# hengdashi/cuda_gcn

Measured on AMD Instinct MI355X. Metric: epochs_per_sec, higher is better.
Workload: dtype f32

## Files before the change

cuda_gcn_amd/_lib.py:

```python
from __future__ import annotations

import ctypes as C
import os

HERE = os.path.dirname(os.path.abspath(__file__))
LIBDIR = os.environ.get("GCN_LIBDIR") or os.path.join(HERE, "lib")

_cache = {}


class NativeLibraryMissing(RuntimeError):
    pass


def _load(name: str) -> C.CDLL:
    if name in _cache:
        return _cache[name]
    path = os.path.join(LIBDIR, name)
    if not os.path.exists(path):
        raise NativeLibraryMissing(
            f"{path} not found: the HIP extension is not built. Run `make kernels host` "
            f"(or __graft_entry__.build()); there is no CPU fallback.")
    try:
        lib = C.CDLL(path)
# ... 33 lines not shown

GCNHIP_SYMBOLS = {
    "gcnhip_device_count": (I, [C.POINTER(I)]),
    "gcnhip_ctx_create": (I, [C.POINTER(P), I, P]),
    "gcnhip_ctx_destroy": (I, [P]),
    "gcnhip_ctx_sync": (I, [P]),
    "gcnhip_ctx_set_corun": (I, [P, I]),
    "gcnhip_ctx_set_option": (I, [P, C.c_char_p, I]),
    "gcnhip_ctx_get_option": (I, [P, C.c_char_p, C.POINTER(I)]),
    "gcnhip_ctx_stream": (P, [P]),
    "gcnhip_error_string": (C.c_char_p, [I]),
    "gcnhip_last_error": (C.c_char_p, []),
    "gcnhip_version": (C.c_char_p, []),
    "gcnhip_experiments": (I, []),
    "gcnhip_malloc": (I, [P, C.POINTER(P), C.c_size_t]),
    "gcnhip_free": (I, [P, P]),
    "gcnhip_memset_async": (I, [P, P, I, C.c_size_t]),
    "gcnhip_h2d": (I, [P, P, P, C.c_size_t]),
    "gcnhip_d2h": (I, [P, P, P, C.c_size_t]),
    "gcnhip_d2d_async": (I, [P, P, P, C.c_size_t]),
    "gcnhip_host_alloc": (I, [C.POINTER(P), C.c_size_t]),
    "gcnhip_host_free": (I, [P]),
    "gcnhip_d2h_async": (I, [P, P, P, C.c_size_t]),
    "gcnhip_graph_create": (I, [P, C.POINTER(P), P, P, I, I, P]),
    "gcnhip_graph_create_grouped": (I, [P, C.POINTER(P), P, P, I, I, P, P]),
    "gcnhip_graph_set_schedule": (I, [P, P, I, P, I]),
    "gcnhip_graph_reserve_width": (I, [P, P, I]),
    "gcnhip_graph_destroy": (I, [P, P]),
    "gcnhip_graph_arrays": (I, [P, C.POINTER(P), C.POINTER(P), C.POINTER(P), C.POINTER(I), C.POINTER(I)]),
    "gcnhip_graphsum": (I, [P, P, P, I, P, I, I]),
    "gcnhip_graphsum_rowmask": (I, [P, P, P, I, P, I, I, P]),
    "gcnhip_graphsum_masked": (I, [P, P, P, I, P, I, I, P, P]),
    "gcnhip_graph_add_rowset": (I, [P, P, P, C.POINTER(P)]),
    "gcnhip_graph_create_restricted": (I, [P, C.POINTER(P), P, P]),
    "gcnhip_graph_clone": (I, [P, C.POINTER(P), P]),
    "gcnhip_rowset_size": (I, [P, C.POINTER(I)]),
    "gcnhip_graphsum_rowset": (I, [P, P, P, P, I, P, I, I, P]),
    "gcnhip_graphsum_relu_dropout": (I, [P, P, P, I, P, I, I, I, F, U64, P, U64, P]),
    "gcnhip_graphsum_relu_dropout_bits": (I, [P, P, P, I, P, I, I, I, F, U64, P, U64, P, P, I]),
    "gcnhip_graphsum_ex": (I, [P, P, P, P, I, P, I, I]),
    "gcnhip_graphsum_predict": (I, [P, P, P, P, P, I, P, I, I, I, P, P, P, I]),
    "gcnhip_graphsum_blend": (I, [P, P, P, I, P, I, P, I, I, F, F, F, F, P]),
    "gcnhip_cs_error_rows": (I, [P, P, I, P, I, P, I, I, P, I, P]),
    "gcnhip_cs_correct_rows": (I, [P, P, I, P, I, P, I, I, P, P, I]),
    "gcnhip_calib_nll_rows": (I, [P, P, I, P, I, P, I, I, F, P]),
    "gcnhip_calib_bins_rows": (I, [P, P, I, P, I, P, I, I, F, I, P, P, P]),
    "gcnhip_calib_scale_rows": (I, [P, P, I, I, P, I, I, F, P, I, P]),
    "gcnhip_conformal_scores": (I, [P, P, I, I, P, I, I, F, I, F, I, P, I]),
    "gcnhip_conformal_true_scores": (I, [P, P, I, P, I, P, I, I, P]),
    "gcnhip_conformal_sets_rows": (I, [P, P, I, I, P, I, I, P, P, P, P, P]),
    "gcnhip_sort_tile": (I, []),
    "gcnhip_rank_keys": (I, [P, P, I, I, P, I, I, I, I, P, P, I, P, P, I64, P, P, P, P]),
    "gcnhip_sort_segments_u32": (I, [P, P, P, I, I, I64]),
    "gcnhip_rank_stats": (I, [P, P, P, I64, I, I, P, P, P, P, P]),
    "gcnhip_embed_inv_norms": (I, [P, P, I, I, I, P]),
    "gcnhip_topk_plan": (I, [I, I, I, I, C.POINTER(I), C.POINTER(I), C.POINTER(C.c_size_t), C.POINTER(C.c_size_t)]),
    "gcnhip_topk_rows": (I, [P, P, I, I, I, P, P, P, I, I, I, I, P, C.c_size_t, I, P, P]),
    "gcnhip_pair_scores": (I, [P, P, I, I, I, P, P, P, I, P]),
    "gcnhip_embed_rows": (I, [P, P, I, I, I, P, P, I, P, I]),
    "gcnhip_explain_hops": (I, [P, P, P, P, I, P, I, I, P, I, I, I, P, P, I, P, P, P, I64]),
    "gcnhip_explain_features_agg": (I, [P, P, P, P, I, P, I, I, P, I, I, P, I, I, P, I, I, P, I]),
    "gcnhip_explain_features_walk": (I, [P, P, P, P, P, I, P, I, I, P, I, I, P, I, I, P, I]),
    "gcnhip_explain_abs_colsum": (I, [P, P, I, P, I, I, I, P, P]),
    "gcnhip_graph_remove_rowset": (I, [P, P, P]),
    "gcnhip_graph_scales": (I, [P, C.POINTER(P), C.POINTER(P), C.POINTER(P), C.POINTER(P)]),
    "gcnhip_feat_scale_rows": (I, [P, P, P]),
    "gcnhip_xent_fwd_rows_scaled": (I, [P, P, I, P, I, P, P, I, I, I, I, I, P, P, P]),
    "gcnhip_xent_from_row_terms": (I, [P, P, P, P, I, P, P]),
    "gcnhip_matmul_bwd_ex": (I, [P, P, I, P, I, P, I, P, I, P, I, I, I, I, F, P, I, P]),
    "gcnhip_graphsum_part": (I, [P, P, P, P, I, P, I, I, P, I, I, I, F, U64, P, U64, P]),
    "gcnhip_feat_create": (I, [P, C.POINTER(P), P, P, P, I, I]),
    "gcnhip_feat_create_aggregated": (I, [P, C.POINTER(P), P, P]),
    "gcnhip_feat_destroy": (I, [P, P]),
    "gcnhip_feat_is_dense": (I, [P]),
    "gcnhip_feat_values": (P, [P]),
    "gcnhip_feat_nnz": (I64, [P]),
    "gcnhip_spmm_fwd": (I, [P, P, P, P, I, P, I, I, F, U64, P, U64, P]),
    "gcnhip_spmm_fwd_relu": (I, [P, P, P, P, I, P, I, I]),
    "gcnhip_spmm_fwd_relu_matmul": (I, [P, P, P, P, I, I, P, I, I, P, I]),
    "gcnhip_spmm_bwd": (I, [P, P, P, P, I, P, I, I, F, U64, P, U64, P]),
    "gcnhip_spmm_bwd_plan": (I, [P, P, I, C.POINTER(I), C.POINTER(I)]),
    "gcnhip_spmm_bwd_part": (I, [P, P, P, P, I, I, F, U64, P, U64, P, I, I, I]),
    "gcnhip_spmm_bwd_finish": (I, [P, P, P, I, I]),
    "gcnhip_matmul_fwd": (I, [P, P, I, P, I, P, I, I, I, I]),
    "gcnhip_matmul_bwd": (I, [P, P, I, P, I, P, I, P, I, P, I, I, I, I]),
    "gcnhip_matmul_bwd_fused": (I, [P, P, I, P, I, P, I, P, I, P, I, I, I, I, F]),
    "gcnhip_matmul_bwd_fused_bits": (I, [P, P, I, P, I, P, I, P, I, P, I, I, I, I, F, P, I]),
    "gcnhip_pack_positive": (I, [P, P, I, I, I, P, I]),
    "gcnhip_f32_to_bf16": (I, [P, P, I, P, I, I64, I]),
    "gcnhip_graphsum_bf16": (I, [P, P, P, I, P, I, I, P, P, I, I, F, U64, P, U64, P]),
    "gcnhip_matmul_bwd_da_bits": (I, [P, P, I, P, I, P, I, I, I, I, P, I, F]),
    "gcnhip_gather_rows": (I, [P, P, I, P, I, P]),
    "gcnhip_relu_fwd": (I, [P, P, P, I64, I]),
    "gcnhip_relu_bwd": (I, [P, P, P, I64]),
    "gcnhip_dropout_fwd": (I, [P, P, P, I64, F, U64, P, U64, P]),
    "gcnhip_dropout_bwd": (I, [P, P, P, I64, F]),
    "gcnhip_relu_fwd_2d": (I, [P, P, I, I, I, P, I]),
    "gcnhip_relu_bwd_2d": (I, [P, P, I, I, I, P]),
    "gcnhip_dropout_fwd_2d": (I, [P, P, I, I, I, P, F, U64, P, U64, P]),
    "gcnhip_dropout_bwd_2d": (I, [P, P, I, I, I, P, F]),
    "gcnhip_relu_dropout_bwd": (I, [P, P, I, P, I, I, I, F]),
    "gcnhip_xent_fwd": (I, [P, P, I, P, I, P, I, I, I, I, I, P, P]),
    "gcnhip_xent_fwd_rows": (I, [P, P, I, P, I, P, P, I, I, I, I, I, P, P]),
    "gcnhip_accuracy": (I, [P, P, I, P, I, I, P]),
    "gcnhip_set_truth": (I, [P, P, P, P, I, I]),
    "gcnhip_sumsq": (I, [P, P, I64, P]),
    "gcnhip_adam_step": (I, [P, C.POINTER(AdamVar), I, F, P, P, F, F, F, F, P]),
    "gcnhip_adam_step_advance": (I, [P, C.POINTER(AdamVar), I, F, P, P, F, F, F, F, P, P, P]),
    "gcnhip_counter_add": (I, [P, P, C.c_uint32]),
    "gcnhip_metrics_record": (I, [P, P, I, I, P, P, P, P]),
    "gcnhip_metrics_record_with_next_loss": (I, [P, P, I, I, P, P]),
    "gcnhip_capture_begin": (I, [P]),
    "gcnhip_capture_end": (I, [P, C.POINTER(P)]),
    "gcnhip_graph_launch": (I, [P, P]),
    "gcnhip_graph_exec_destroy": (I, [P]),
    "gcnhip_event_create": (I, [C.POINTER(P)]),
    "gcnhip_event_create_sync": (I, [C.POINTER(P)]),
    "gcnhip_event_destroy": (I, [P]),
    "gcnhip_event_record": (I, [P, P]),
    "gcnhip_stream_wait_event": (I, [P, P]),
    "gcnhip_event_elapsed_ms": (I, [P, P, C.POINTER(F)]),
    "gcnhip_event_sync": (I, [P]),
    "gcnhip_bce_fwd_rows": (I, [P, P, I, P, I, P, I, P, I, I, I, I, P, P, P]),
    "gcnhip_bce_predict_rows": (I, [P, P, I, P, I, I, P, I, P, I]),
    "gcnhip_confusion_rows": (I, [P, P, P, I, P, I, I, P, P]),
    "gcnhip_bce_class_counts_rows": (I, [P, P, I, P, I, P, I, I, P]),
    "gcnhip_wxent_fwd_rows": (I, [P, P, I, P, I, P, P, I, I, I, I, I, P, P, P, P, F]),
    "gcnhip_wbce_fwd_rows": (I, [P, P, I, P, I, P, I, P, I, I, I, I, P, P, P, P]),
}


def _declare_gcnhip(lib):
    for name, (res, args) in GCNHIP_SYMBOLS.items():
        fn = getattr(lib, name)
        fn.restype = res
        fn.argtypes = args


class HostParams(C.Structure):
    _fields_ = [("num_nodes", I), ("input_dim", I), ("hidden_dim", I), ("output_dim", I),
                ("dropout", F), ("learning_rate", F), ("weight_decay", F), ("epochs", I), ("early_stopping", I)]


ALLGATHER_FN = C.CFUNCTYPE(None, P, C.POINTER(C.c_float), C.c_size_t)
ALLREDUCE_FN = C.CFUNCTYPE(None, P, C.POINTER(C.c_double), C.c_size_t)
PP = C.POINTER(P)

GCNHOST_SYMBOLS = {
    "gcnhost_last_error": (C.c_char_p, []),
    "gcnhost_params_default": (HostParams, []),
    "gcnhost_nccl_unique_id": (I, [C.c_char_p]),
    "gcnhost_model_create": (I, [PP, C.POINTER(HostParams), P, P, P, P, P, P, P, C.c_long, I, I, I, I, C.c_char_p,
                                 ALLGATHER_FN, ALLREDUCE_FN, P]),
    "gcnhost_model_create_multilabel": (I, [PP, C.POINTER(HostParams), P, P, P, P, P, P, P, P, C.c_long, I, I, I, I, C.c_char_p,
                                            ALLGATHER_FN, ALLREDUCE_FN, P]),
    "gcnhost_model_create_weighted": (I, [PP, C.POINTER(HostParams), P, P, P, P, P, P, P, P, P, C.c_long, I, I, I, I, C.c_char_p,
                                          ALLGATHER_FN, ALLREDUCE_FN, P]),
    "gcnhost_balanced_class_weights": (I, [I, I, P, P, P, I, P]),
    "gcnhost_class_weights_read": (I, [C.c_char_p, C.POINTER(I), P]),
    "gcnhost_model_destroy": (I, [P]),
    "gcnhost_model_train_epoch": (I, [P, C.POINTER(F), C.POINTER(F)]),
    "gcnhost_model_eval": (I, [P, I, C.POINTER(F), C.POINTER(F)]),
    "gcnhost_model_run_epochs": (I, [P, I, P]),
    "gcnhost_model_run": (I, [P]),
    "gcnhost_model_sync": (I, [P]),
    "gcnhost_model_info": (I, [P, C.POINTER(I), C.POINTER(I), C.POINTER(I), C.POINTER(I), C.POINTER(I64)]),
# ... 68 lines not shown
```

cuda_gcn_amd/csrc/common.h:

```cpp
#pragma once
#include <memory>
#include <vector>
#include <hip/hip_runtime.h>
#include <stdint.h>
#include <stddef.h>
#include "devbuf.h"
#include "../../include/gcnhip_driver.h"

#define GCNHIP_TRY(expr)                                   \
    do {                                                   \
        hipError_t _e = (expr);                            \
        if (_e != hipSuccess) return (int)_e;              \
    } while (0)
#define GCNHIP_LAUNCH_CHECK() GCNHIP_TRY(hipGetLastError())

constexpr int WAVE = 64;

int gcnhip_fail(const char *detail);

struct GcnOptions {
    int gs_u;
    int gs_l;
    int gemm_bf16x3;
    int spmm_slices;
    int xent_finalize;
    int adam_sum_launch;
    int spmm_general;
    int spmm_rows;
    int spmm_nw;
    int split_edges;
};
struct GcnOptionEntry { const char *name; int GcnOptions::*field; int dflt; };
extern const GcnOptionEntry GCN_OPTION_TABLE[];
extern const int GCN_OPTION_COUNT;

struct gcnhip_ctx {
    int device = 0;
    GcnOptions opt = {};
    hipStream_t stream = nullptr;
    bool own_stream = false;
    int n_cu = 0;
    DevBuf<float> red_f;
    DevBuf<int32_t> red_i;
    DevBuf<uint32_t> ticket;
    bool rec_armed = false;
    float *rec_ring = nullptr; int rec_capacity = 0, rec_slot = 0; const uint32_t *rec_epoch = nullptr; const float *rec_sumsq = nullptr;
    DevBuf<float> slab;
    size_t slab_bytes = 0;
    int slab_n = 0;
    DevBuf<float> wpack;
    size_t wpack_bytes = 0;
    int corun = 0;
};
constexpr size_t WPACK_BYTES = (size_t)2 << 20;
constexpr int RED_SLOTS = 4096;

struct gcnhip_graph;
struct gcnhip_rowset {
    const gcnhip_graph *owner = nullptr;
    std::vector<uint32_t> bits;
    int n_tasks = 0;
    DevBuf<int4> tasks;
    int n_split_rows = 0;
    DevBuf<int4> split_rows;
    int bounds[4][9] = {};
};

struct gcnhip_graph {
    int n_rows = 0, n_cols = 0, nnz = 0;
    DevBuf<int> indptr;
    DevBuf<int> indices;
    DevBuf<float> coef;
    DevBuf<float> dinv_row, dinv2_row;
    DevBuf<float> dinv_col, dinv2_col;
    int split_edges_opt = 0;
    int n_tasks = 0;
    DevBuf<int4> tasks;
    int n_split_rows = 0;
    DevBuf<int4> split_rows;
    DevBuf<float> partials;
    int part_ld = 0;
    int n_slots = 0;
    int bounds[4][9] = {};
    std::vector<int> h_indptr;
    std::vector<int4> h_tasks, h_srows;
    std::vector<std::unique_ptr<gcnhip_rowset>> rowsets;
};

struct gcnhip_feat {
    int n_rows = 0, n_cols = 0;
    int64_t nnz = 0;
    bool dense = false;
    DevBuf<int> indptr;
    DevBuf<int> indices;
    DevBuf<float> values;
    DevBuf<float> values_pad;
    int ld_pad = 0;
    DevBuf<int> csc_ptr;
    DevBuf<int> csc_row;
    DevBuf<int> csc_pos;
    DevBuf<float> csc_val;
    DevBuf<uint32_t> keep_bits;
    int keep_layout = 0;
    DevBuf<int4> bwd_tasks;
    int n_bwd_tasks = 0, bwd_nw = 0;
    DevBuf<int4> bwd_split;
    int n_bwd_split = 0, n_bwd_slots = 0;
    DevBuf<float> bwd_partials;
    int bwd_part_ld = 0;
};

static inline int upload_lists(const std::vector<int4> &tasks, const std::vector<int4> &split, DevBuf<int4> &d_tasks, DevBuf<int4> &d_split) {
    d_tasks.reset();
    d_split.reset();
    if (!tasks.empty()) GCNHIP_TRY(d_tasks.upload(tasks.data(), tasks.size()));
    if (!split.empty()) GCNHIP_TRY(d_split.upload(split.data(), split.size()));
    return 0;
}

__host__ __device__ inline void philox4x32_10(uint32_t c0, uint32_t c1, uint32_t c2, uint32_t c3,
                                              uint32_t k0, uint32_t k1, uint32_t out[4]) {
    const uint32_t M0 = 0xD2511F53u, M1 = 0xCD9E8D57u, W0 = 0x9E3779B9u, W1 = 0xBB67AE85u;
#pragma unroll
    for (int r = 0; r < 10; r++) {
        const uint64_t p0 = (uint64_t)M0 * c0, p1 = (uint64_t)M1 * c2;
        const uint32_t n0 = (uint32_t)(p1 >> 32) ^ c1 ^ k0;
        const uint32_t n1 = (uint32_t)p1;
        const uint32_t n2 = (uint32_t)(p0 >> 32) ^ c3 ^ k1;
        const uint32_t n3 = (uint32_t)p0;
        c0 = n0; c1 = n1; c2 = n2; c3 = n3;
        k0 += W0; k1 += W1;
    }
    out[0] = c0; out[1] = c1; out[2] = c2; out[3] = c3;
}

__host__ __device__ inline int dropout_threshold(float p) {
    int t = (int)(p * 65536.0f + 0.5f);
    return t < 0 ? 0 : (t > 65535 ? 65535 : t);
}

__device__ inline uint32_t keep_word(uint64_t c, int g, uint32_t epoch, uint64_t seed, int thr16) {
    if (thr16 == 0) return 0xFFFFFFFFu;
    const int n_planes = 16 - (__ffs(thr16) - 1);
    uint32_t ge = 0xFFFFFFFFu;
    for (int i = n_planes; i >= 1; i--) {
        uint32_t r[4];
        philox4x32_10((uint32_t)c, (uint32_t)(c >> 32), epoch, (uint32_t)i, (uint32_t)seed, (uint32_t)(seed >> 32), r);
        const uint32_t P = g == 0 ? r[0] : (g == 1 ? r[1] : (g == 2 ? r[2] : r[3]));
        ge = (thr16 >> (16 - i) & 1) ? (P & ge) : (P | ge);
    }
    return ge;
}
__device__ inline bool keep1(uint64_t j, uint32_t epoch, uint64_t seed, int thr16) {
    return (keep_word(j >> 7, (int)(j >> 5) & 3, epoch, seed, thr16) >> (j & 31)) & 1u;
}
template <int V>
__device__ inline uint32_t keepv(uint64_t j, uint32_t epoch, uint64_t seed, int thr16) {
    return (keep_word(j >> 7, (int)(j >> 5) & 3, epoch, seed, thr16) >> (j & 31)) & ((1u << V) - 1u);
}
__device__ inline uint32_t keep4(uint64_t quad, uint32_t epoch, uint64_t seed, int thr16) {
    return keepv<4>(quad << 2, epoch, seed, thr16);
}

__device__ inline float wave_sum(float v) {
#pragma unroll
    for (int off = 32; off > 0; off >>= 1) v += __shfl_xor(v, off, WAVE);
    return v;
}
__device__ inline int wave_sum_i(int v) {
#pragma unroll
    for (int off = 32; off > 0; off >>= 1) v += __shfl_xor(v, off, WAVE);
    return v;
}

struct RingRow {
    float *ring; int capacity, slot; const uint32_t *epoch; const float *sumsq;
};
__device__ inline void ring_row_write(const RingRow &g, float r0, float r1, float r2, float r3) {
    if (!g.ring) return;
    const uint32_t e = g.epoch ? *g.epoch : 0u;
    float *row = g.ring + ((size_t)(e % (uint32_t)g.capacity) * 4 + g.slot) * 8;
    row[0] = r0; row[1] = r1; row[2] = r2; row[3] = r3;
    row[4] = g.sumsq ? *g.sumsq : 0.f;
    row[5] = (float)e; row[6] = 0.f; row[7] = 0.f;
}
static inline RingRow ring_row_take(gcnhip_ctx *c) {
// ... 23 lines not shown
```

cuda_gcn_amd/csrc/dense_bf16x3.h:

```cpp
#pragma once
#include "dense_persist.h"
#include "bf16x3_split.h"

constexpr int BX_BK = 32;
constexpr int BX_BH_BYTES = 3 * 4 * 1024;
constexpr int BX_NB = 10;
constexpr int BX_PD = 6;
constexpr int BX_SMEM = BX_NB * BX_BH_BYTES;


__device__ inline void bx_pack_w_body(int idx, const float *__restrict__ w, int ldw, int K, int n_hs, uint4 *__restrict__ wp, float scale) {
    if (idx >= n_hs * 4 * 64) return;
    const int lane = idx & 63, n = (idx >> 6) & 3, hs = idx >> 8;
    const int col = 32 * n + (lane & 31), k0 = 32 * (hs >> 1) + 16 * (lane >> 5) + 8 * (hs & 1);
    BxPlanes P;
#pragma unroll
    for (int i = 0; i < 4; i++) {
        const int k = k0 + 2 * i;
        const float a = k < K ? w[(size_t)k * ldw + col] * scale : 0.f, b = (k + 1) < K ? w[(size_t)(k + 1) * ldw + col] * scale : 0.f;
        bx_split2(a, b, P.w[0][i], P.w[1][i], P.w[2][i]);
    }
#pragma unroll
    for (int p = 0; p < 3; p++) wp[(((size_t)hs * 3 + p) * 4 + n) * 64 + lane] = make_uint4(P.w[p][0], P.w[p][1], P.w[p][2], P.w[p][3]);
}
__device__ inline void bx_pack_w2_body(int idx, const float *__restrict__ w2, int ldw2, int p2, uint4 *__restrict__ img) {
    if (idx >= 8 * 2 * 64) return;
    const int ln = idx & 63, cb = (idx >> 6) & 1, s = idx >> 7;
    const int c = 32 * cb + (ln & 31), h = ln >> 5;
    BxPlanes P;
#pragma unroll
    for (int i = 0; i < 4; i++) {
        float v[2];
#pragma unroll
        for (int u = 0; u < 2; u++) {
            const int j = 2 * i + u;
            const int f = 32 * (s >> 1) + (j & 3) + 8 * ((j >> 2) + 2 * (s & 1)) + 4 * h;
            v[u] = c < p2 ? w2[(size_t)f * ldw2 + c] : 0.f;
        }
        bx_split2(v[0], v[1], P.w[0][i], P.w[1][i], P.w[2][i]);
    }
#pragma unroll
    for (int p = 0; p < 3; p++) img[((s * 2 + cb) * 3 + p) * 64 + ln] = make_uint4(P.w[p][0], P.w[p][1], P.w[p][2], P.w[p][3]);
}
__global__ __launch_bounds__(256) void bx_pack_w_kernel(const float *__restrict__ w, int ldw, int K, int n_hs, uint4 *__restrict__ wp, float scale,
                                                        const float *__restrict__ w2 = nullptr, int ldw2 = 0, int p2 = 0, uint4 *__restrict__ img = nullptr) {
    if ((int)blockIdx.x < n_hs) bx_pack_w_body(blockIdx.x * blockDim.x + threadIdx.x, w, ldw, K, n_hs, wp, scale);
    else bx_pack_w2_body(((int)blockIdx.x - n_hs) * 256 + threadIdx.x, w2, ldw2, p2, img);
}
struct BxBitsArgs {
    uint32_t *bits; int m, K, n_chunks, R;
    int thr; uint64_t seed; const uint32_t *d_epoch; uint64_t off; const uint8_t *keep_mask;
};
constexpr int BX_BITS_LDS_WORDS = 4096;
__device__ inline void dropbits_cm_body(int wg, int tid, const BxBitsArgs &b, uint32_t *lds) {
    const int ra = wg * b.R, rb = min(b.m, ra + b.R);
    if (ra >= rb) return;
    const uint64_t bit0 = b.off + (uint64_t)ra * b.K;
    const uint64_t q0 = bit0 >> 7;
    if (!b.keep_mask) {
        const uint64_t bit1 = b.off + (uint64_t)rb * b.K + 64;
        const int n_blk = (int)((bit1 >> 7) - q0) + 1;
        const uint32_t epoch = b.d_epoch ? *b.d_epoch : 0u;
        for (int blk = tid; blk < n_blk; blk += 256) {
            const uint64_t c = q0 + (uint64_t)blk;
            uint32_t ge[4] = {0xFFFFFFFFu, 0xFFFFFFFFu, 0xFFFFFFFFu, 0xFFFFFFFFu};
            if (b.thr != 0) {
                const int n_planes = 16 - (__ffs(b.thr) - 1);
                for (int i = n_planes; i >= 1; i--) {
                    uint32_t r[4];
                    philox4x32_10((uint32_t)c, (uint32_t)(c >> 32), epoch, (uint32_t)i, (uint32_t)b.seed, (uint32_t)(b.seed >> 32), r);
                    const bool and_plane = (b.thr >> (16 - i)) & 1;
#pragma unroll
                    for (int g = 0; g < 4; g++) ge[g] = and_plane ? (r[g] & ge[g]) : (r[g] | ge[g]);
                }
            }
#pragma unroll
            for (int g = 0; g < 4; g++) lds[4 * blk + g] = ge[g];
        }
    }
    __syncthreads();
    const int rows = rb - ra;
    const uint32_t rel0 = (uint32_t)(bit0 - (q0 << 7));
    for (int idx = tid; idx < b.n_chunks * rows; idx += 256) {
        int c, r;
        if (rows == 128) { c = idx >> 7; r = idx & 127; } else { c = idx / rows; r = idx - c * rows; }
        const int row = ra + r;
        const int valid = min(32, b.K - 32 * c);
        uint32_t word;
        if (b.keep_mask) {
            word = 0;
            const uint8_t *km = b.keep_mask + (size_t)row * b.K + 32 * c;
            for (int i = 0; i < valid; i++) word |= (km[i] ? 1u : 0u) << i;
        } else {
            const uint32_t rel = rel0 + (uint32_t)r * (uint32_t)b.K + 32u * (uint32_t)c;
            const uint32_t lo = lds[rel >> 5], hi = lds[(rel >> 5) + 1], sh = rel & 31u;
            word = sh ? ((lo >> sh) | (hi << (32u - sh))) : lo;
            if (valid < 32) word &= (1u << valid) - 1u;
        }
        b.bits[(size_t)c * b.m + row] = word;
    }
}
__global__ __launch_bounds__(256) void dropbits_cm_kernel(BxBitsArgs b) {
    __shared__ uint32_t lds[BX_BITS_LDS_WORDS];
    dropbits_cm_body(blockIdx.x, threadIdx.x, b, lds);
}
__global__ __launch_bounds__(256) void dropbits_bx_pack_w_kernel(BxBitsArgs b, int n_bits_wgs,
                                                                 const float *__restrict__ w, int ldw, int K, int n_hs,
                                                                 uint4 *__restrict__ wp, float scale) {
    __shared__ uint32_t lds[BX_BITS_LDS_WORDS];
    if ((int)blockIdx.x < n_bits_wgs) dropbits_cm_body(blockIdx.x, threadIdx.x, b, lds);
    else bx_pack_w_body(((int)blockIdx.x - n_bits_wgs) * 256 + threadIdx.x, w, ldw, K, n_hs, wp, scale);
}

struct Bx3FwdArgs {
    const float *x; int ldx;
    const uint4 *wp;
    float *out; int ldo;
    int m, K, n_chunks, n_rb;
    const uint32_t *bits;
    int relu;
    const uint4 *w2p;
    float *z0; int ldz, p2;
};
constexpr int BX_W2_BYTES = 8 * 2 * 3 * 1024;

struct BxB3 { bf16x8 h, m, l; };
template <int N> struct BxN { static constexpr int value = N; };
struct BxRaw { f32x4 v[4]; uint32_t kw; };

template <int OFF>
__device__ __forceinline__ void bx_gload16(f32x4 &dst, const float *p) {
    asm volatile("global_load_dwordx4 %0, %1, off offset:%2" : "=v"(dst) : "v"(p), "n"(OFF) : "memory");
}
__device__ __forceinline__ void bx_gload4(uint32_t &dst, const uint32_t *p) {
    asm volatile("global_load_dword %0, %1, off" : "=v"(dst) : "v"(p) : "memory");
}
template <int OFF>
__device__ __forceinline__ void bx_ldsread16(bf16x8 &dst, uint32_t addr) {
    asm volatile("ds_read_b128 %0, %1 offset:%2" : "=v"(dst) : "v"(addr), "n"(OFF) : "memory");
}
#define BX_WAIT_LDS(b) asm volatile("s_waitcnt lgkmcnt(0)" : "+v"((b).h), "+v"((b).m), "+v"((b).l) :: "memory")
#define BX_PIN(P, i) asm volatile("" : "+v"((P).w[0][i]), "+v"((P).w[1][i]), "+v"((P).w[2][i]))
#define BX_WAIT_RAW(N, r) asm volatile("s_waitcnt vmcnt(" #N ")" : "+v"((r).v[0]), "+v"((r).v[1]), "+v"((r).v[2]), "+v"((r).v[3]), "+v"((r).kw) :: "memory")

template <bool DROP, int NP, bool ZOUT = false>
// ... 483 lines not shown
```

cuda_gcn_amd/csrc/feat.hip:

```cpp
#include "common.h"
#include "plan.h"

extern "C" {

__global__ void feat_scale_rows_kernel(float *vals, float *vals_pad, int ld_pad, const int *indptr, const float *scale, int n_rows, int n_cols, int dense) {
    const int r = blockIdx.x * (blockDim.x >> 6) + (threadIdx.x >> 6);
    if (r >= n_rows) return;
    const float s = scale[r];
    const int lane = threadIdx.x & 63;
    for (int e = indptr[r] + lane; e < indptr[r + 1]; e += 64) vals[e] *= s;
    if (vals_pad && dense)
        for (int k = lane; k < n_cols; k += 64) vals_pad[(size_t)r * ld_pad + k] *= s;
}
__global__ void feat_scale_csc_kernel(float *csc_val, const int *csc_row, const float *scale, int64_t nnz) {
    const int64_t q = (int64_t)blockIdx.x * blockDim.x + threadIdx.x;
    if (q < nnz) csc_val[q] *= scale[csc_row[q]];
}
int gcnhip_feat_scale_rows(gcnhip_ctx *c, gcnhip_feat *f, const float *d_row_scale) {
    if (!c || !f || !d_row_scale) return -1;
    if (f->n_rows == 0) return 0;
    feat_scale_rows_kernel<<<ceil_div(f->n_rows, 4), 256, 0, c->stream>>>(f->values, f->values_pad, f->ld_pad, f->indptr, d_row_scale, f->n_rows, f->n_cols, f->dense ? 1 : 0);
    GCNHIP_LAUNCH_CHECK();
    if (f->csc_val && f->nnz) {
        feat_scale_csc_kernel<<<ceil_div(f->nnz, 256), 256, 0, c->stream>>>(f->csc_val, f->csc_row, d_row_scale, f->nnz);
        GCNHIP_LAUNCH_CHECK();
    }
    GCNHIP_TRY(hipStreamSynchronize(c->stream));
    return 0;
}

int gcnhip_feat_create(gcnhip_ctx *c, gcnhip_feat **out, const int *h_indptr, const int *h_indices,
                       const float *h_values, int n_rows, int n_cols) {
    if (!c || !out || !h_indptr || !h_values || n_rows < 0 || n_cols <= 0) return -1;
    GCNHIP_TRY(hipSetDevice(c->device));
    std::unique_ptr<gcnhip_feat> f(new gcnhip_feat());
    f->n_rows = n_rows; f->n_cols = n_cols;
    const int64_t nnz = h_indptr[n_rows];
    f->nnz = nnz;
    const bool dense = plan::dense_layout(h_indptr, h_indices, n_rows, n_cols);
    if (!h_indices && !dense) return -1;
    f->dense = dense;
    GCNHIP_TRY(f->indptr.upload(h_indptr, (size_t)n_rows + 1));
    GCNHIP_TRY(f->values.alloc((size_t)std::max<int64_t>(nnz, 4)));
    if (nnz) GCNHIP_TRY(hipMemcpy(f->values, h_values, (size_t)nnz * sizeof(float), hipMemcpyHostToDevice));
    {
        const size_t words_cm = dense ? (size_t)n_rows * ((n_cols + 31) / 32) : 0;
        GCNHIP_TRY(f->keep_bits.alloc(std::max((size_t)(nnz / 32), words_cm) + 32));
    }
    if (dense && n_cols % 128 != 0 && n_cols >= 64) {
        f->ld_pad = (n_cols + 127) / 128 * 128;
        GCNHIP_TRY(f->values_pad.alloc((size_t)n_rows * f->ld_pad));
        GCNHIP_TRY(hipMemset(f->values_pad, 0, (size_t)n_rows * f->ld_pad * sizeof(float)));
        GCNHIP_TRY(hipMemcpy2D(f->values_pad, (size_t)f->ld_pad * sizeof(float), f->values, (size_t)n_cols * sizeof(float),
                               (size_t)n_cols * sizeof(float), (size_t)n_rows, hipMemcpyDeviceToDevice));
    }
    if (!dense) {
        if (!plan::indices_in_range(h_indices, nnz, n_cols)) return -1;
        GCNHIP_TRY(f->indices.upload(h_indices, (size_t)nnz));
        const plan::Csc csc = plan::csc_sort(h_indptr, h_indices, n_rows, n_cols);
        GCNHIP_TRY(f->csc_ptr.upload(csc.ptr.data(), csc.ptr.size()));
        GCNHIP_TRY(f->csc_row.upload(csc.row.data(), (size_t)nnz));
        GCNHIP_TRY(f->csc_pos.upload(csc.pos.data(), (size_t)nnz));
        if (nnz) {
            std::vector<float> cv((size_t)nnz);
            for (int64_t q = 0; q < nnz; q++) cv[q] = h_values[csc.pos[q]];
            GCNHIP_TRY(f->csc_val.upload(cv.data(), (size_t)nnz));
        }
        f->bwd_nw = plan::column_waves(nnz, n_cols, c->opt.spmm_nw);
        const plan::Schedule s = plan::cut_segments(csc.ptr.data(), nullptr, n_cols, plan::column_segment(f->bwd_nw));
        f->n_bwd_tasks = (int)s.tasks.size(); f->n_bwd_split = (int)s.split.size(); f->n_bwd_slots = s.n_slots;
        GCNHIP_TRY((hipError_t)upload_lists(s.tasks, s.split, f->bwd_tasks, f->bwd_split));
    }
    *out = f.release();
    return 0;
}

int gcnhip_feat_create_aggregated(gcnhip_ctx *c, gcnhip_feat **out, gcnhip_graph *g, const gcnhip_feat *x) {
    if (!c || !out || !g || !x || !x->dense || x->n_rows != g->n_cols) return -1;
    GCNHIP_TRY(hipSetDevice(c->device));
    std::unique_ptr<gcnhip_feat> f(new gcnhip_feat());
    const int F = x->n_cols, n = g->n_rows;
    f->n_rows = n; f->n_cols = F; f->nnz = (int64_t)n * F; f->dense = true;
    std::vector<int> ip((size_t)n + 1);
    for (int r = 0; r <= n; r++) ip[r] = (int)((int64_t)r * F);
    GCNHIP_TRY(f->indptr.upload(ip.data(), (size_t)n + 1));
    GCNHIP_TRY(f->values.alloc((size_t)std::max<int64_t>(f->nnz, 4)));
    int rc = gcnhip_graph_reserve_width(c, g, F);
    if (rc != 0) return rc;
    const float *src = x->values_pad ? x->values_pad : x->values;
    const int ld_src = x->values_pad ? x->ld_pad : F;
    if (x->values_pad) {
        f->ld_pad = x->ld_pad;
        GCNHIP_TRY(f->values_pad.alloc((size_t)n * f->ld_pad));
        GCNHIP_TRY(hipMemsetAsync(f->values_pad, 0, (size_t)n * f->ld_pad * sizeof(float), c->stream));
        rc = gcnhip_graphsum(c, g, src, ld_src, f->values_pad, f->ld_pad, F);
        if (rc != 0) return rc;
        GCNHIP_TRY(hipMemcpy2DAsync(f->values, (size_t)F * sizeof(float), f->values_pad, (size_t)f->ld_pad * sizeof(float),
                                    (size_t)F * sizeof(float), (size_t)n, hipMemcpyDeviceToDevice, c->stream));
    } else {
        rc = gcnhip_graphsum(c, g, src, ld_src, f->values, F, F);
        if (rc != 0) return rc;
    }
    GCNHIP_TRY(hipStreamSynchronize(c->stream));
    *out = f.release();
    return 0;
}

int gcnhip_feat_destroy(gcnhip_ctx *c, gcnhip_feat *f) {
    if (!f) return 0;
    hipSetDevice(c->device);
    delete f;
    return 0;
}
int gcnhip_feat_is_dense(const gcnhip_feat *f) { return f && f->dense ? 1 : 0; }
const float *gcnhip_feat_values(const gcnhip_feat *f) { return f ? f->values : nullptr; }
int64_t gcnhip_feat_nnz(const gcnhip_feat *f) { return f ? f->nnz : 0; }

}
```

cuda_gcn_amd/csrc/spmm.hip:

```cpp
#include "dense_kernels.h"
#include "dense_tile128.h"
#include "dense_persist.h"
#include "dense_bf16x3.h"
#include "spmm_sparse.h"
#include <limits.h>

struct DenseFwdArgs {
    const float *x; int ldx;
    const float *w; int ldw;
    float *out; int ldo;
    int m, K, p;
    const uint32_t *bits;
    float scale;
    int relu;
};

constexpr int DF_BM = 128, DF_BK = 32;
constexpr int DF_ALD = DF_BK + 2;

template <int NT, int VX>
__global__ __launch_bounds__(256) void spmm_dense_fwd_kernel(DenseFwdArgs a) {
    constexpr int BN = NT * 16;
    constexpr int BLD = BN + 16;
    __shared__ __attribute__((aligned(16))) float As[DF_BM * DF_ALD];
// ... 48 lines not shown
            for (int s = 0; s < VX; s++)
                As[r * DF_ALD + c + s] = a.bits ? ((kb >> s & 1u) ? areg[pc][s] * a.scale : 0.f) : areg[pc][s];
        }
#pragma unroll
        for (int pc = 0; pc < B_PIECES; pc++) {
            const int idx = (pc * 256 + tid) * 4;
            const int k = idx / BN, c = idx % BN;
            if (k < DF_BK) {
#pragma unroll
                for (int s = 0; s < 4; s++) Bs[k * BLD + c + s] = breg[pc][s];
            }
        }
    };

    f32x4 acc[2][NT];
#pragma unroll
    for (int r = 0; r < 2; r++)
#pragma unroll
        for (int t = 0; t < NT; t++) acc[r][t] = (f32x4){0.f, 0.f, 0.f, 0.f};

    fetch(0);
    for (int k0 = 0; k0 < a.K; k0 += DF_BK) {
        __syncthreads();
        stash(k0);
        __syncthreads();
        if (k0 + DF_BK < a.K) fetch(k0 + DF_BK);
#pragma unroll
        for (int kk = 0; kk < DF_BK; kk += 4) {
            float af[2], bf[NT];
#pragma unroll
            for (int r = 0; r < 2; r++) af[r] = As[(wave * 32 + r * 16 + li) * DF_ALD + kk + kq];
#pragma unroll
            for (int t = 0; t < NT; t++) bf[t] = Bs[(kk + kq) * BLD + t * 16 + li];
#pragma unroll
            for (int r = 0; r < 2; r++)
#pragma unroll
                for (int t = 0; t < NT; t++)
                    acc[r][t] = __builtin_amdgcn_mfma_f32_16x16x4f32(af[r], bf[t], acc[r][t], 0, 0, 0);
        }
    }
#pragma unroll
    for (int r = 0; r < 2; r++)
#pragma unroll
        for (int t = 0; t < NT; t++) {
            const int col = col_base + t * 16 + li;
            if (col >= a.p) continue;
#pragma unroll
            for (int i = 0; i < 4; i++) {
                const int row = row_base + wave * 32 + r * 16 + 4 * kq + i;
                if (row < a.m) a.out[(size_t)row * a.ldo + col] = (a.relu && !(acc[r][t][i] > 0.f)) ? 0.f : acc[r][t][i];
            }
        }
}

constexpr int64_t SPMM_NARROW_MIN_NNZ = 262144;

static DropSpec make_drop(float p_drop, uint64_t seed, const uint32_t *d_epoch, uint64_t off, const uint8_t *keep_mask) {
    DropSpec d;
    d.on = p_drop > 0.f || keep_mask != nullptr;
    d.thr = dropout_threshold(p_drop);
    d.scale = 1 / (1 - p_drop);
    d.seed = seed; d.off = off; d.d_epoch = d_epoch; d.keep_mask = keep_mask;
    return d;
}

static inline bool keep_bits_by_block(const DropSpec &d) { return !d.keep_mask && (d.off & 127) == 0; }

static int make_keep_bits(gcnhip_ctx *c, const gcnhip_feat *f, const DropSpec &d) {
    if (!f->keep_bits) return gcnhip_fail("input dropout on a feature object without a keep-bit array (gcnhip_feat_create_aggregated builds evaluation-only objects)");
    const_cast<gcnhip_feat *>(f)->keep_layout = 0;
    const int64_t words = (f->nnz + 31) / 32;
    if (keep_bits_by_block(d))
        dropbits_block_kernel<<<ceil_div((words + 3) / 4, 256), 256, 0, c->stream>>>(f->keep_bits, f->nnz, d.thr, d.seed, d.d_epoch, d.off >> 7);
    else
        dropbits_kernel<<<ceil_div(words, 256), 256, 0, c->stream>>>(f->keep_bits, f->nnz, d.thr, d.seed, d.d_epoch, d.off, d.keep_mask);
    GCNHIP_LAUNCH_CHECK();
    return 0;
}

static BxBitsArgs keep_bits_cm_args(const gcnhip_feat *f, const DropSpec &d) {
    BxBitsArgs b;
    b.bits = f->keep_bits; b.m = f->n_rows; b.K = f->n_cols; b.n_chunks = (f->n_cols + 31) / 32;
    b.R = std::max(1, std::min(128, (BX_BITS_LDS_WORDS - 12) * 32 / std::max(1, f->n_cols)));
    b.thr = d.thr; b.seed = d.seed; b.d_epoch = d.d_epoch; b.off = d.off; b.keep_mask = d.keep_mask;
    return b;
}
static inline bool keep_bits_cm_fit(const gcnhip_feat *f) { return f->dense && f->keep_bits && f->n_cols / 32 + 16 <= BX_BITS_LDS_WORDS; }
static int make_keep_bits_cm(gcnhip_ctx *c, const gcnhip_feat *f, const DropSpec &d) {
    if (!keep_bits_cm_fit(f)) return gcnhip_fail("chunk-major keep bits: not a dense feature object with a keep-bit array");
    const BxBitsArgs b = keep_bits_cm_args(f, d);
    const_cast<gcnhip_feat *>(f)->keep_layout = 1;
    dropbits_cm_kernel<<<ceil_div(b.m, b.R), 256, 0, c->stream>>>(b);
    GCNHIP_LAUNCH_CHECK();
    return 0;
}
static int want_keep_layout(gcnhip_ctx *c, const gcnhip_feat *f, const DropSpec &d, int layout, bool fresh = false) {
    if (!d.on || (!fresh && f->keep_layout == layout)) return 0;
    return layout ? make_keep_bits_cm(c, f, d) : make_keep_bits(c, f, d);
}

static int x_vec_width(const gcnhip_feat *f, const float *vals) {
    return (f->n_cols % 4 == 0 && aligned16(vals)) ? 4 : ((f->n_cols % 2 == 0 && ((uintptr_t)vals & 7) == 0) ? 2 : 1);
}

template <int NT>
static void launch_dense_fwd(const DenseFwdArgs &a, int vx, dim3 grid, hipStream_t s) {
    if (vx == 4) spmm_dense_fwd_kernel<NT, 4><<<grid, 256, 0, s>>>(a);
    else if (vx == 2) spmm_dense_fwd_kernel<NT, 2><<<grid, 256, 0, s>>>(a);
    else spmm_dense_fwd_kernel<NT, 1><<<grid, 256, 0, s>>>(a);
}

extern "C" {

struct Z0Fuse { const float *w2; int ld_w2, p2; float *z0; int ld_z0; };

constexpr int NOT_MINE = INT_MIN;

static bool dense_fwd_bf16x3_fits(const gcnhip_ctx *c, const gcnhip_feat *f, const Tile128Args &t, const DropSpec &d, bool fast, bool fused) {
    const int n_chunks = (t.K + PG_BK - 1) / PG_BK;
    return fast && t.p == 128 && c->opt.gemm_bf16x3 && (!d.on || keep_bits_cm_fit(f)) &&
           (fused || ((c->opt.gemm_bf16x3 >= 2 || !c->corun) && aligned16(t.out) && (uint64_t)(t.m + 256) * (uint64_t)t.ldo * 4u < (1ull << 32))) &&
           aligned16(t.x) && (size_t)n_chunks * 2 * BX_BH_BYTES <= c->wpack_bytes;
}
static bool dense_fwd_bf16x3_z0_fits(const gcnhip_ctx *c, const Tile128Args &t, const DropSpec &d, bool fast, const Z0Fuse &zf) {
    const int n_chunks = (t.K + PG_BK - 1) / PG_BK;
    return fast && t.p == 128 && c->opt.gemm_bf16x3 && !d.on && aligned16(t.x) && zf.p2 >= 1 && zf.p2 <= 64 && zf.ld_z0 % 4 == 0 &&
           zf.ld_z0 >= zf.p2 && zf.ld_w2 >= zf.p2 && aligned16(zf.z0) && (size_t)n_chunks * 2 * BX_BH_BYTES + BX_W2_BYTES <= c->wpack_bytes;
}
static int dense_fwd_bf16x3(gcnhip_ctx *c, const gcnhip_feat *f, const Tile128Args &t, const DropSpec &d, bool fast, const Z0Fuse *zf) {
    if (zf && !dense_fwd_bf16x3_z0_fits(c, t, d, fast, *zf)) return GCNHIP_NOT_AVAILABLE;
    if (!dense_fwd_bf16x3_fits(c, f, t, d, fast, zf != nullptr)) return NOT_MINE;
    const int n_chunks = (t.K + PG_BK - 1) / PG_BK, n_hs = 2 * n_chunks;
    uint4 *wp3 = reinterpret_cast<uint4 *>((float *)c->wpack);
    uint4 *w2img = wp3 + (size_t)n_hs * (BX_BH_BYTES / 16);
    if (d.on) {
        const BxBitsArgs kb = keep_bits_cm_args(f, d);
        const int n_bits_wgs = ceil_div(kb.m, kb.R);
        const_cast<gcnhip_feat *>(f)->keep_layout = 1;
        dropbits_bx_pack_w_kernel<<<n_bits_wgs + n_hs, 256, 0, c->stream>>>(kb, n_bits_wgs, t.w, t.ldw, t.K, n_hs, wp3, t.scale);
    } else {
        if (zf) bx_pack_w_kernel<<<n_hs + 4, 256, 0, c->stream>>>(t.w, t.ldw, t.K, n_hs, wp3, 1.f, zf->w2, zf->ld_w2, zf->p2, w2img);
        else bx_pack_w_kernel<<<n_hs, 256, 0, c->stream>>>(t.w, t.ldw, t.K, n_hs, wp3, t.bits ? t.scale : 1.f);
    }
    GCNHIP_LAUNCH_CHECK();
    Bx3FwdArgs ba;
    ba.x = t.x; ba.ldx = t.ldx; ba.wp = wp3; ba.out = t.out; ba.ldo = t.ldo;
    ba.m = t.m; ba.K = t.K; ba.n_chunks = n_chunks; ba.n_rb = ceil_div(t.m, 32);
    ba.bits = t.bits; ba.relu = t.relu;
    ba.w2p = nullptr; ba.z0 = nullptr; ba.ldz = 0; ba.p2 = 0;
    const int wgs = std::max(1, std::min(c->n_cu, ba.n_rb));
    if (zf) {
        ba.w2p = w2img; ba.z0 = zf->z0; ba.ldz = zf->ld_z0; ba.p2 = zf->p2;
        dense_fwd_bf16x3_kernel<false, 6, true><<<wgs, 512, 0, c->stream>>>(ba);
    } else if (ba.bits) {
        dense_fwd_bf16x3_kernel<true, 6><<<wgs, 512, 0, c->stream>>>(ba);
    } else {
        dense_fwd_bf16x3_kernel<false, 6><<<wgs, 512, 0, c->stream>>>(ba);
    }
    GCNHIP_LAUNCH_CHECK();
    return 0;
}

static bool dense_fwd_persist_fits(const gcnhip_ctx *c, const Tile128Args &t, bool fast) {
    const int n_chunks = (t.K + PG_BK - 1) / PG_BK;
    return fast && t.p == 128 && !c->corun && aligned16(t.x) && aligned16(t.out) &&
           (uint64_t)(t.m + PG_ROWS) * (uint64_t)t.ldo * 4u < (1ull << 32) && (size_t)n_chunks * 4096 * sizeof(float) <= c->wpack_bytes;
}
static int dense_fwd_persist(gcnhip_ctx *c, const gcnhip_feat *f, const Tile128Args &t, const DropSpec &d, bool fast) {
    if (!dense_fwd_persist_fits(c, t, fast)) return NOT_MINE;
    const int n_chunks = (t.K + PG_BK - 1) / PG_BK;
    if (d.on && keep_bits_by_block(d)) {
        const int n_bits_wgs = (int)ceil_div(((f->nnz + 31) / 32 + 3) / 4, (int64_t)256);
        const_cast<gcnhip_feat *>(f)->keep_layout = 0;
        dropbits_pack_w_kernel<<<n_bits_wgs + n_chunks * 4, 256, 0, c->stream>>>(f->keep_bits, f->nnz, d.thr, d.seed, d.d_epoch, d.off >> 7, n_bits_wgs,
                                                                               t.w, t.ldw, t.K, n_chunks * 4, c->wpack, t.scale);
    } else {
        if (d.on) { const int rc = make_keep_bits(c, f, d); if (rc) return rc; }
        pg_pack_w_kernel<<<ceil_div(n_chunks * 4 * 256, 256), 256, 0, c->stream>>>(t.w, t.ldw, t.K, n_chunks * 4, c->wpack, t.bits ? t.scale : 1.f);
    }
    GCNHIP_LAUNCH_CHECK();
    PersistFwdArgs pa;
    pa.x = t.x; pa.ldx = t.ldx; pa.wp = c->wpack; pa.out = t.out; pa.ldo = t.ldo;
    pa.m = t.m; pa.K = t.K; pa.n_chunks = n_chunks; pa.n_rb = ceil_div(t.m, 32);
    pa.bits = t.bits; pa.relu = t.relu;
    const int wgs = std::max(1, std::min(c->n_cu, pa.n_rb));
    if (pa.bits) dense_fwd_persist_kernel<true><<<wgs, 512, 0, c->stream>>>(pa);
    else dense_fwd_persist_kernel<false><<<wgs, 512, 0, c->stream>>>(pa);
    GCNHIP_LAUNCH_CHECK();
    return 0;
}

static int dense_fwd_tiles(gcnhip_ctx *c, const gcnhip_feat *f, const Tile128Args &t, const DropSpec &d, bool fast, int vx) {
    if (d.on) { const int rc = make_keep_bits(c, f, d); if (rc) return rc; }
    const dim3 grid(ceil_div(t.m, T_BM), ceil_div(t.p, T_BN));
    if (fast) dense_fwd_t128w8_kernel<<<grid, 512, 0, c->stream>>>(t);
    else if (vx == 4) dense_fwd_t128_kernel<4><<<grid, 256, 0, c->stream>>>(t);
    else if (vx == 2) dense_fwd_t128_kernel<2><<<grid, 256, 0, c->stream>>>(t);
    else dense_fwd_t128_kernel<1><<<grid, 256, 0, c->stream>>>(t);
    GCNHIP_LAUNCH_CHECK();
    return 0;
}

static int spmm_fwd_impl(gcnhip_ctx *c, const gcnhip_feat *f, const float *vals, const float *w, int ld_w,
                         float *out, int ld_out, int p, float p_drop, uint64_t seed, const uint32_t *d_epoch,
                         uint64_t nnz_offset, const uint8_t *keep_mask, int relu, const Z0Fuse *zf = nullptr) {
    if (!c || !f || !vals || !w || (!out && !zf) || p <= 0 || ld_w < p || (out && ld_out < p)) return -1;
    if (!(p_drop >= 0.f && p_drop < 1.f)) return -1;
    if (zf && !(f->dense && p == 128)) return GCNHIP_NOT_AVAILABLE;
    if (f->n_rows == 0) return 0;
    const DropSpec d = make_drop(p_drop, seed, d_epoch, nnz_offset, keep_mask);
    if (f->dense && p > 64) {
        if (d.on && !f->keep_bits) return gcnhip_fail("input dropout on a feature object without a keep-bit array (gcnhip_feat_create_aggregated builds evaluation-only objects)");
        Tile128Args t;
        t.x = vals; t.ldx = f->n_cols; t.w = w; t.ldw = ld_w; t.out = out; t.ldo = ld_out;
        int vx = x_vec_width(f, vals);
        if (vals == f->values && f->values_pad) { t.x = f->values_pad; t.ldx = f->ld_pad; vx = 4; }
        t.m = f->n_rows; t.K = f->n_cols; t.p = p; t.bits = d.on ? f->keep_bits : nullptr; t.scale = d.scale; t.rows_per_split = 0; t.relu = relu;
        const bool fast = vx == 4 && t.ldx % 4 == 0 && (t.K + 31) / 32 * 32 <= t.ldx && ld_w % 4 == 0 && p % T_BN == 0 && aligned16(w);
        int rc = dense_fwd_bf16x3(c, f, t, d, fast, zf);
        if (rc == NOT_MINE) rc = dense_fwd_persist(c, f, t, d, fast);
        if (rc == NOT_MINE) rc = dense_fwd_tiles(c, f, t, d, fast, vx);
        return rc;
    }
    if (f->dense) {
        if (d.on) { const int rc = make_keep_bits(c, f, d); if (rc) return rc; }
        DenseFwdArgs a;
        a.x = vals; a.ldx = f->n_cols; a.w = w; a.ldw = ld_w; a.out = out; a.ldo = ld_out;
        a.m = f->n_rows; a.K = f->n_cols; a.p = p; a.bits = d.on ? f->keep_bits : nullptr; a.scale = d.scale; a.relu = relu;
        int vx = x_vec_width(f, vals);
        if (vals == f->values && f->values_pad) { a.x = f->values_pad; a.ldx = f->ld_pad; vx = 4; }
        const int nt_total = ceil_div(p, 16);
        const int NT = nt_total >= 8 ? 8 : (nt_total > 4 ? 8 : (nt_total > 2 ? 4 : nt_total));
        dim3 grid(ceil_div(f->n_rows, DF_BM), ceil_div(nt_total, NT));
        switch (NT) {
            case 1: launch_dense_fwd<1>(a, vx, grid, c->stream); break;
            case 2: launch_dense_fwd<2>(a, vx, grid, c->stream); break;
            case 4: launch_dense_fwd<4>(a, vx, grid, c->stream); break;
            default: launch_dense_fwd<8>(a, vx, grid, c->stream); break;
        }
        GCNHIP_LAUNCH_CHECK();
        return 0;
    }
    SpFwdArgs a;
    a.indptr = f->indptr; a.indices = f->indices; a.vals = vals; a.w = w; a.out = out;
    a.n_rows = f->n_rows; a.ld_w = ld_w; a.ld_out = ld_out; a.p = p; a.d = d; a.relu = relu;
    a.w_floats = f->n_cols * ld_w;
    a.rows_per_wave = 1;
    const bool vec = ld_w % 4 == 0 && aligned16(w);
    const int units = vec ? (p + 3) / 4 : p;
    a.nnz_bytes = (int)std::min<int64_t>(f->nnz * 4, 0x7FFFFFFF);
    a.rows_per_wave = std::max(1, std::min(8, (int)(f->n_rows / ((int64_t)c->n_cu * 64))));
    if (c->opt.spmm_rows > 0) a.rows_per_wave = std::min(32, c->opt.spmm_rows);
    a.n_slices = 1;
    if (vec && c->opt.spmm_slices != 0 && p % 32 == 0 && (p / 32 == 2 || p / 32 == 4 || p / 32 == 8) &&
        (size_t)f->n_cols * ld_w * sizeof(float) > ((size_t)4 << 20) && f->n_rows >= 8 * 64) {
        a.n_slices = p / 32;
        if (c->opt.spmm_rows <= 0) a.rows_per_wave = 2;
        const int Gs = 8 / a.n_slices;
        const int units_total = ceil_div(f->n_rows, a.rows_per_wave);
        const int per_group = ceil_div(units_total, Gs) + 1;
        dim3 sgrid(8 * ceil_div(per_group, 4), 1);
        a.nnz_bytes = (int)std::min<int64_t>(f->nnz * 4, 0x7FFFFFFF);
        spmm_csr_fwd_kernel<8, true, true><<<sgrid, 256, 0, c->stream>>>(a);
        GCNHIP_LAUNCH_CHECK();
        return 0;
    }
    dim3 grid(ceil_div(ceil_div(f->n_rows, a.rows_per_wave), 4), 1);
    a.nnz_bytes = (int)std::min<int64_t>(f->nnz * 4, 0x7FFFFFFF);
    const bool narrow = vec && units <= 16 && f->nnz * 4 < 0x7FFFFFFF && c->opt.spmm_general <= 0 && (f->nnz >= SPMM_NARROW_MIN_NNZ || c->opt.spmm_general < 0);
    if (narrow) {
        if (units <= 1) spmm_csr_fwd_q_kernel<1><<<grid, 256, 0, c->stream>>>(a);
        else if (units <= 2) spmm_csr_fwd_q_kernel<2><<<grid, 256, 0, c->stream>>>(a);
        else if (units <= 4) spmm_csr_fwd_q_kernel<4><<<grid, 256, 0, c->stream>>>(a);
        else if (units <= 8) spmm_csr_fwd_q_kernel<8><<<grid, 256, 0, c->stream>>>(a);
        else spmm_csr_fwd_q_kernel<16><<<grid, 256, 0, c->stream>>>(a);
        GCNHIP_LAUNCH_CHECK();
        return 0;
    }
#define SPF(L_)                                                                           \
    do {                                                                                  \
        if (vec) spmm_csr_fwd_kernel<L_, true><<<grid, 256, 0, c->stream>>>(a);           \
        else spmm_csr_fwd_kernel<L_, false><<<grid, 256, 0, c->stream>>>(a);              \
    } while (0)
    if (units <= 1) SPF(1); else if (units <= 2) SPF(2); else if (units <= 4) SPF(4);
    else if (units <= 8) SPF(8); else if (units <= 16) SPF(16); else if (units <= 32) SPF(32); else SPF(64);
#undef SPF
    GCNHIP_LAUNCH_CHECK();
    return 0;
}

int gcnhip_spmm_fwd(gcnhip_ctx *c, const gcnhip_feat *f, const float *vals, const float *w, int ld_w,
                    float *out, int ld_out, int p, float p_drop, uint64_t seed, const uint32_t *d_epoch,
                    uint64_t nnz_offset, const uint8_t *keep_mask) {
    return spmm_fwd_impl(c, f, vals, w, ld_w, out, ld_out, p, p_drop, seed, d_epoch, nnz_offset, keep_mask, 0);
}

int gcnhip_spmm_fwd_relu(gcnhip_ctx *c, const gcnhip_feat *f, const float *vals, const float *w, int ld_w,
                         float *out, int ld_out, int p) {
    return spmm_fwd_impl(c, f, vals, w, ld_w, out, ld_out, p, 0.f, 0, nullptr, 0, nullptr, 1);
}

int gcnhip_spmm_fwd_relu_matmul(gcnhip_ctx *c, const gcnhip_feat *f, const float *vals, const float *w, int ld_w, int p,
                                const float *w2, int ld_w2, int p2, float *z0, int ld_z0) {
    if (!w2 || !z0 || p2 <= 0) return -1;
    const Z0Fuse zf = {w2, ld_w2, p2, z0, ld_z0};
    return spmm_fwd_impl(c, f, vals, w, ld_w, nullptr, 0, p, 0.f, 0, nullptr, 0, nullptr, 1, &zf);
}

static bool dense_bwd_plan(const gcnhip_ctx *c, const gcnhip_feat *f, int p, int *rps_out, int *S_out) {
    if (!(f->dense && p > 64 && f->n_cols >= 64)) return false;
    const int kt = ceil_div(f->n_cols, 128), pt = ceil_div(p, 128);
    int S = (2 * c->n_cu) / (kt * pt);
    if (S < 1) S = 1;
    int rps = (ceil_div(f->n_rows, S) + T_BK - 1) / T_BK * T_BK;
    if (rps < T_BK) rps = T_BK;
    *rps_out = rps;
    *S_out = ceil_div(f->n_rows, rps);
    return true;
}
static bool dense_bwd_bf16x3_fits(const gcnhip_ctx *c, const gcnhip_feat *f, const float *vals, const float *dout, int ld_dout, int p,
                                  const DropSpec &d, int rps) {
    const int bx = c->opt.gemm_bf16x3, kt = ceil_div(f->n_cols, 128);
    const bool padded = vals == f->values && f->values_pad && f->ld_pad >= kt * 128;
    return bx && (bx >= 2 || !c->corun) && p == 128 && padded && rps % 16 == 0 && ld_dout % 4 == 0 && aligned16(dout) &&
           (uint64_t)f->n_rows * (uint64_t)f->ld_pad * 4u < (1ull << 32) && (uint64_t)f->n_rows * (uint64_t)ld_dout * 4u < (1ull << 32) &&
           (uint64_t)f->n_rows * (uint64_t)f->n_cols < (1ull << 32) && (uint64_t)kt * 16u * (uint64_t)f->n_rows < (1ull << 32) &&
           (!d.on || keep_bits_cm_fit(f));
}

static int dense_bwd_part(gcnhip_ctx *c, const gcnhip_feat *f, const float *vals, const float *dout, int ld_dout, int p,
                          const DropSpec &d, int s0, int s1, bool fresh) {
    int rps, S;
    if (!dense_bwd_plan(c, f, p, &rps, &S) || s0 < 0 || s1 > S || s0 > s1) return -1;
    if (s0 == s1) return 0;
    if (d.on && !f->keep_bits) return gcnhip_fail("input dropout on a feature object without a keep-bit array");
    c->slab_n = S;
    const int kt = ceil_div(f->n_cols, 128), pt = ceil_div(p, 128);
    const int p_ld = (p + 3) / 4 * 4;
    const int rc = ensure_slab(c, (size_t)S * f->n_cols * p_ld * sizeof(float));
    if (rc) return rc;
    if (dense_bwd_bf16x3_fits(c, f, vals, dout, ld_dout, p, d, rps)) {
        { const int rl = want_keep_layout(c, f, d, 1, fresh); if (rl) return rl; }
        Bx3BwdArgs b;
        b.x = f->values_pad; b.ldx = f->ld_pad; b.dout = dout; b.ldd = ld_dout; b.slab = c->slab; b.p_ld = p_ld;
        b.m = f->n_rows; b.K = f->n_cols; b.rps = rps; b.split0 = s0; b.bits = d.on ? f->keep_bits : nullptr; b.scale = d.on ? d.scale : 1.f;
        const dim3 grid(kt, s1 - s0);
        if (b.bits) dense_bwd_bf16x3_kernel<true, 6><<<grid, 256, 0, c->stream>>>(b);
        else dense_bwd_bf16x3_kernel<false, 6><<<grid, 256, 0, c->stream>>>(b);
        GCNHIP_LAUNCH_CHECK();
        return 0;
    }
    { const int rl = want_keep_layout(c, f, d, 0, fresh); if (rl) return rl; }
    Tile128Args t;
    t.x = vals; t.ldx = f->n_cols; t.w = dout; t.ldw = ld_dout; t.out = c->slab; t.ldo = p_ld;
    int vx = x_vec_width(f, vals);
    if (vals == f->values && f->values_pad) { t.x = f->values_pad; t.ldx = f->ld_pad; vx = 4; }
    t.m = f->n_rows; t.K = f->n_cols; t.p = p; t.bits = d.on ? f->keep_bits : nullptr; t.scale = d.scale; t.rows_per_split = rps; t.relu = 0;
    t.split0 = s0;
    dim3 grid(s1 - s0, kt, pt);
    const bool fast = vx == 4 && t.ldx % 4 == 0 && kt * 128 <= t.ldx && ld_dout % 4 == 0 && p % 128 == 0 && aligned16(dout);
    if (fast) dense_bwd_t128_kernel<4, true><<<grid, 256, 0, c->stream>>>(t);
    else if (vx == 4) dense_bwd_t128_kernel<4><<<grid, 256, 0, c->stream>>>(t);
    else if (vx == 2) dense_bwd_t128_kernel<2><<<grid, 256, 0, c->stream>>>(t);
    else dense_bwd_t128_kernel<1><<<grid, 256, 0, c->stream>>>(t);
    GCNHIP_LAUNCH_CHECK();
    return 0;
}

static int dense_bwd_finish(gcnhip_ctx *c, const gcnhip_feat *f, float *dw, int ld_dw, int p) {
    int rps, S;
    if (!dense_bwd_plan(c, f, p, &rps, &S)) return -1;
    const int p_ld = (p + 3) / 4 * 4;
    const int n_slabs = c->slab_n > 0 ? c->slab_n : S;
    if (!c->slab || c->slab_bytes < (size_t)n_slabs * f->n_cols * p_ld * sizeof(float)) return -1;
    launch_slab_reduce(c->slab, n_slabs, f->n_cols, p, p_ld, dw, ld_dw, c->stream);
    GCNHIP_LAUNCH_CHECK();
    return 0;
}

int gcnhip_spmm_bwd_plan(const gcnhip_ctx *c, const gcnhip_feat *f, int p, int *rows_per_split, int *n_splits) {
    if (!c || !f || p <= 0 || !rows_per_split || !n_splits) return -1;
    int rps = 0, S = 0;
    if (!dense_bwd_plan(c, f, p, &rps, &S)) { rps = 0; S = 0; }
    *rows_per_split = rps; *n_splits = S;
    return 0;
}

int gcnhip_spmm_bwd_part(gcnhip_ctx *c, const gcnhip_feat *f, const float *vals, const float *dout, int ld_dout, int p,
                         float p_drop, uint64_t seed, const uint32_t *d_epoch, uint64_t nnz_offset, const uint8_t *keep_mask,
// ... 86 lines not shown
```

cuda_gcn_amd/host/gcn.h:

```cpp
#pragma once
#include <memory>
#include <utility>
#include <vector>
#include "comm.h"
#include "device_arena.h"
#include "module.h"
#include "optim.h"
#include "partition.h"
#include "sparse.h"
#include "timer.h"
#include "variable.h"

struct GCNParams {
    int num_nodes, input_dim, hidden_dim, output_dim;
    float dropout, learning_rate, weight_decay;
    int epochs, early_stopping;
    static GCNParams get_default();
};

class GCNData {
public:
    SparseIndex feature_index, graph;
    std::vector<int> split;
    std::vector<int> label;
// ... 146 lines not shown
    const float *full_vals = nullptr;
    bool replicate_l1 = false;
    bool rebuild_dh1 = false;
    uint32_t *d_pos_bits = nullptr;
    std::vector<std::unique_ptr<HipVariable>> variables;
    HipVariable *input = nullptr, *output = nullptr;
    const float *input_vals = nullptr;
    std::vector<Module *> modules;
    std::unique_ptr<HipAdam> optimizer;

    float *gradbuf = nullptr;
    size_t gradbuf_elems = 0;
    float *d_result = nullptr;
    int32_t *d_result_i = nullptr;
    int32_t *d_truth[4] = {};
    ScoredSplit scored;
    void fill_scored(ScoredSplit &d, int s, gcnhip_rowset *const *rows) const;
    uint32_t *d_ml_truth = nullptr;
    int ml_wpr = 0;
    std::pair<float, float> ring_metrics(const float *row) const;
    friend class ModelQueries;
    std::unique_ptr<ModelQueries> queries_;
    void forward_hooked(const HipGraphSum::Prediction *prediction, const HipGraphSum::Redirect *redirect);
    bool forward_hidden_only();
    gcnhip_graph *graph_bwd_out = nullptr;
    gcnhip_graph *graph_loc = nullptr, *graph_rem = nullptr, *graph_bwd_loc = nullptr, *graph_bwd_rem = nullptr;
    gcnhip_rowset *split_rows_loc[4] = {}, *split_rows_rem[4] = {};
    std::unique_ptr<ExchangeLane> xlane;
    void build_overlap();
    void wire_overlap(HipGraphSum *gs, bool output_layer);
    std::vector<uint32_t> h_train_bits;
    uint32_t *d_train_bits = nullptr;
    const uint32_t *bwd_bits = nullptr;
    gcnhip_rowset *split_rows[4] = {};
    int32_t *d_split_list[4] = {};
    int split_local_n[4] = {};
    int split_count[4] = {};
    float *d_class_w = nullptr;
    float split_wsum[4] = {};
    float *d_ring = nullptr;
    static constexpr int RING = 1024;
    uint8_t *d_keep0 = nullptr, *d_keep1 = nullptr;
    std::vector<uint8_t> h_keep0, h_keep1;
    long keep0_first = 0;
    long epochs_done = 0;
    void *epoch_graph = nullptr;
    bool enqueue_epoch_replay();
    bool zipped() const { return lane && !(timers->enabled && env.comm->size() == 1); }
    void enqueue_epoch(bool first, bool last);
    void print_line(long epoch, std::pair<float, float> train, std::pair<float, float> scored_now, float dt) const;
    static constexpr int PIPELINE_DEPTH = 4;
    static constexpr int READBACK_GROUP_MAX = 64;
    static constexpr int READBACK_CALIBRATION = 16;
    static constexpr double READBACK_GROUP_SECONDS = 2e-3;
    struct Readback {
        gcnhip_ctx *ctx = nullptr;
        float *host = nullptr;
        void *ev_ready[PIPELINE_DEPTH] = {}, *ev_copied[PIPELINE_DEPTH] = {};
    };
    std::unique_ptr<Readback> readback;
    void readback_create(bool own_stream);
    void readback_destroy();
    void readback_enqueue(long first_epoch_index, int n_epochs, int slot, gcnhip_ctx *producer);
    void run_synchronous();
    void run_pipelined();
    void report_test();

    struct EvalLane {
        HipEnv env;
        DeviceArena arena;
        ExchangeBuffers xbuf;
        std::unique_ptr<Comm> comm;
        std::unique_ptr<DeviceTimers> timers;
        gcnhip_graph *graph = nullptr;
        gcnhip_graph *graph_l1 = nullptr;
        std::unique_ptr<HipVariable> H0, H1, Z0, Z;
        std::vector<Module *> modules;
        float *d_result = nullptr;
        int32_t *d_result_i = nullptr;
        gcnhip_rowset *split_rows[4] = {};
        ScoredSplit scored;
        void *ev_weights = nullptr, *ev_done = nullptr;
        void *ev_fork = nullptr;
        bool pending = false;
        long epoch_word = -1;
    };
    std::unique_ptr<EvalLane> lane;
    void init(const HipGCNOptions &opt);
    void release();
    void destroy_lane();
    void build_eval_lane();
    void eval_on_lane(int current_split);
    void lane_begin(int current_split);
    void lane_end(int current_split);
    void eval_then_train_zipped(int current_split);
    void train_begin();
    void train_end();
    void refresh_input();
    void metrics_before(HipEnv &e, int slot, const uint32_t *epoch_word);
    void metrics_after(HipEnv &e, DeviceTimers &t, int slot, const uint32_t *epoch_word, float *result, size_t n);
    gcnhip_graph *create_rows_graph(gcnhip_ctx *ctx);

    int sched_mode = 0, sched_groups = 0, slice_floats = 64;
    bool labels_assortative = false;
    std::vector<int> structure_group;
    int structure_n_groups = 0;
    void tune_schedule();
    void choose_slice_width();
    void apply_schedule(gcnhip_ctx *ctx, gcnhip_graph *g);
    void add_split_rowsets(gcnhip_ctx *ctx, gcnhip_graph *g, gcnhip_rowset *out[4]);
    void build_modules();
    struct LossSite {
        HipEnv *env;
        HipVariable *Z;
        const ScoredSplit *split;
        float *d_result;
        int32_t *d_result_i;
        bool shift_in_place;
        const float *grad_row_scale;
        bool list_rows;
        HipGraphSum *epilogue;
    };
    Module *make_loss(const LossSite &s);
    void set_truth(int current_split);
    void host_masks_for_epoch();
    void train_epoch_async();
    void eval_async(int current_split);
    std::pair<float, float> read_metrics(long epoch_index, int slot);
};
```

cuda_gcn_amd/host/gcn_build.cpp:

```cpp
#include "gcn.h"
#include "queries.h"
#include "class_weights.h"
#include "cluster.h"
#include <chrono>
#include <future>
#include <cstdio>
#include "hip_check.h"

GCNParams GCNParams::get_default() { return {2708, 1433, 16, 7, 0.5, 0.01, 5e-4, 100, 0}; }

namespace {
bool labels_are_assortative(const GCNData &d, int N, int C) {
    if ((int)d.label.size() != N || C <= 1) return false;
    const std::vector<int> &gp = d.graph.indptr, &gi = d.graph.indices;
    std::vector<double> freq(C, 0.0);
    for (int i = 0; i < N; i++) {
        if (d.label[i] < 0 || d.label[i] >= C) return false;
        freq[d.label[i]] += 1.0;
    }
    double chance = 0;
    for (int c = 0; c < C; c++) chance += (freq[c] / N) * (freq[c] / N);
    long same = 0, total = 0;
    for (int i = 0; i < N; i++)
        for (int e = gp[i]; e < gp[i + 1]; e++) {
// ... 279 lines not shown
    for (int s = 1; s <= 3; s++) {
        std::vector<uint32_t> bits((size_t)n_local / 32 + 2, 0u);
        for (int r = 0; r < n_local; r++)
            if (data->split[r0 + r] == s) bits[r >> 5] |= 1u << (r & 31);
        GCNHIP_CHECK(gcnhip_graph_add_rowset(ctx, g, bits.data(), &out[s]));
    }
}

void HipGCN::build_overlap() {
    const size_t n_pos = (size_t)xplan.table_rows;
    std::vector<uint32_t> own(n_pos / 32 + 2, 0u), other(n_pos / 32 + 2, 0u);
    for (size_t t = 0; t < n_pos; t++) {
        const bool mine = (int)t >= xplan.own_offset && (int)t < xplan.own_offset + n_local;
        (mine ? own : other)[t >> 5] |= 1u << (t & 31);
    }
    xlane.reset(new ExchangeLane(env.ctx, device_, env.comm, xplan, (int)xbuf.max_ld_words, timers->enabled));
    env.xlane = xlane.get();
    if (n_local == 0) return;
    GCNHIP_CHECK(gcnhip_graph_create_restricted(env.ctx, &graph_loc, graph, own.data()));
    GCNHIP_CHECK(gcnhip_graph_create_restricted(env.ctx, &graph_rem, graph, other.data()));
    if (graph_bwd_out) {
        GCNHIP_CHECK(gcnhip_graph_create_restricted(env.ctx, &graph_bwd_loc, graph_bwd_out, own.data()));
        GCNHIP_CHECK(gcnhip_graph_create_restricted(env.ctx, &graph_bwd_rem, graph_bwd_out, other.data()));
    }
    if (!(flags & HIPGCN_ALL_ROWS)) {
        add_split_rowsets(env.ctx, graph_loc, split_rows_loc);
        add_split_rowsets(env.ctx, graph_rem, split_rows_rem);
    }
}

void HipGCN::wire_overlap(HipGraphSum *gs, bool output_layer) {
    if (!graph_loc) return;
    gs->split_loc = graph_loc; gs->split_rem = graph_rem;
    if (!output_layer) return;
    gs->bwd_split_loc = graph_bwd_loc; gs->bwd_split_rem = graph_bwd_rem;
    if (!(flags & HIPGCN_ALL_ROWS)) { gs->fwd_out_rows_loc = &scored.out_rows_loc; gs->fwd_out_rows_rem = &scored.out_rows_rem; }
}

Module *HipGCN::make_loss(const LossSite &s) {
    const int C = params.output_dim;
    if (opt_.multilabel) {
        auto *bce = new HipBCELoss(s.env, s.Z, d_ml_truth, ml_wpr, &s.split->count, s.d_result, s.d_result_i, C);
        bce->rows_list = &s.split->rows; bce->rows_n = &s.split->rows_n; bce->grad_row_scale = s.grad_row_scale;
        bce->d_pos_weight = d_class_w;
        return bce;
    }
    auto *ce = new HipCrossEntropyLoss(s.env, s.Z, &s.split->truth, &s.split->count, s.d_result, s.d_result_i, C, s.shift_in_place);
    if (s.list_rows) { ce->rows_list = &s.split->rows; ce->rows_n = &s.split->rows_n; }
    ce->grad_row_scale = s.grad_row_scale;
    ce->d_weight = d_class_w; ce->weight_sum = &s.split->wsum;
    if (s.epilogue && !d_class_w && opt_.loss_epilogue && C <= 64 && !s.env->bf16_tables) {
        const size_t n = (size_t)2 * std::max(n_local, 1);
        ce->row_terms = (s.env == &env ? arena : lane->arena).upload(std::vector<float>(n, 0.f).data(), n);
        s.epilogue->loss = ce;
    }
    return ce;
}

void HipGCN::build_modules() {
    const int N = n_local, F = params.input_dim, H = params.hidden_dim, C = params.output_dim;
    const int rank = env.comm->rank();
    const uint64_t nnz_off = (uint64_t)data->feature_index.indptr[part.start[rank]];
    const uint64_t hid_off = (uint64_t)part.start[rank] * H;
    HipVariable *H0 = variables[1].get(), *W1 = variables[2].get(), *H1 = variables[3].get(),
                *Z0 = variables[4].get(), *W2 = variables[5].get(), *Z = variables[6].get();
    const float p = params.dropout;
    static const uint8_t *const no_mask = nullptr;
    if (flags & HIPGCN_MODULAR) {
        modules.push_back(new HipDropout(&env, input, p, KEY_INPUT_DROPOUT, nnz_off, (flags & HIPGCN_HOST_MASKS) ? &env.keep_input : &no_mask));
        modules.push_back(new HipSparseMatmul(&env, &input_vals, W1, H0, feat, N, F, H, 0.f, nnz_off));
        { auto *gs = new HipGraphSum(&env, H0, H1, graph, H); wire_overlap(gs, false); modules.push_back(gs); }
        modules.push_back(new HipReLU(&env, H1));
        modules.push_back(new HipDropout(&env, H1, p, KEY_HIDDEN_DROPOUT, hid_off, (flags & HIPGCN_HOST_MASKS) ? &env.keep_hidden : &no_mask));
        modules.push_back(new HipMatmul(&env, H1, W2, Z0, N, H, C));
        { auto *gs = new HipGraphSum(&env, Z0, Z, graph, C); gs->bwd_row_bits = &bwd_bits; gs->bwd_graph = graph_bwd_out; gs->fwd_out_rows = &scored.out_rows; wire_overlap(gs, true); modules.push_back(gs); logits_gs = gs; }
        modules.push_back(make_loss({&env, Z, &scored, d_result, d_result_i, true, nullptr,
                                     opt_.multilabel || d_class_w != nullptr, nullptr}));
    } else {
        const float scale = 1 / (1 - p);
        auto *sm = new HipSparseMatmul(&env, &input_vals, W1, H0, feat, N, F, H, p, nnz_off);
        auto *gs = new HipGraphSum(&env, H0, H1, graph, H, p, hid_off);
        auto *mm = new HipMatmul(&env, H1, W2, Z0, N, H, C, scale);
        if (replicate_l1) { sm->sp_full = feat_full; sm->vals_full = &full_vals; gs->fwd_graph_replicated = graph_l1; }
        wire_overlap(gs, false);
        if (factored_) {
            const float *dinv_row = nullptr, *dinv2_row = nullptr, *dinv2_col = nullptr;
            GCNHIP_CHECK(gcnhip_graph_scales(graph, &dinv_row, &dinv2_row, nullptr, &dinv2_col));
            gs->fwd_scaling = 2; gs->bwd_scaling = 3;
            mm->da_row_scale = dinv2_row;
            mm->da_row_scale_full = dinv2_col;
        }
        if (env.comm->size() == 1 && H % 32 == 0 && !env.bf16_tables && opt_.mask_bits) {
            const int wpr = H / 32;
            d_pos_bits = arena.upload(std::vector<uint32_t>((size_t)N * wpr, 0u).data(), (size_t)N * wpr);
            gs->mask_bits_out = d_pos_bits;
            mm->mask_bits = d_pos_bits; mm->mask_wpr = wpr;
        }
        if (rebuild_dh1) {
            const int wpr = (H + 31) / 32;
            d_pos_bits = arena.upload(std::vector<uint32_t>((size_t)xplan.table_rows * wpr, 0u).data(), (size_t)xplan.table_rows * wpr);
            gs->pos_bits_full = d_pos_bits; gs->wpr = wpr; gs->out_grad_complete = true;
            mm->pos_bits_full = d_pos_bits; mm->wpr = wpr; mm->all_rows = xplan.table_rows;
        }
        modules.push_back(sm);
        modules.push_back(gs);
        modules.push_back(mm);
        HipGraphSum *gs_logits = nullptr;
        {
            auto *gs = new HipGraphSum(&env, Z0, Z, graph, C);
            gs->bwd_row_bits = &bwd_bits; gs->bwd_graph = graph_bwd_out; gs->fwd_out_rows = &scored.out_rows;
            if (factored_) { gs->fwd_scaling = 1; gs->bwd_scaling = 3; }
            wire_overlap(gs, true);
            modules.push_back(gs);
            gs_logits = gs;
            logits_gs = gs;
        }
        const float *dinv = nullptr;
        if (factored_) GCNHIP_CHECK(gcnhip_graph_scales(graph, &dinv, nullptr, nullptr, nullptr));
        modules.push_back(make_loss({&env, Z, &scored, d_result, d_result_i, false, dinv, true, gs_logits}));
    }
}

gcnhip_graph *HipGCN::create_rows_graph(gcnhip_ctx *ctx) {
    const std::vector<int> &gp = data->graph.indptr, &gi = data->graph.indices;
    const int N = params.num_nodes, r0 = part.start[env.comm->rank()];
    std::vector<int> lp(n_local + 1), deg(N);
    for (int r = 0; r <= n_local; r++) lp[r] = gp[r0 + r] - gp[r0];
    for (int j = 0; j < N; j++) deg[j] = gp[j + 1] - gp[j];
    gcnhip_graph *g = nullptr;
    GCNHIP_CHECK(gcnhip_graph_create(ctx, &g, lp.data(), gi.data() + gp[r0], n_local, N, deg.data()));
    const int rc = gcnhip_graph_reserve_width(ctx, g, std::max(params.hidden_dim, params.output_dim));
    if (rc != 0) gcnhip_graph_destroy(ctx, g);
    GCNHIP_CHECK(rc);
    return g;
}

void HipGCN::build_agg_first_eval() {
    const int world = env.comm->size();
    const int N = params.num_nodes, F = params.input_dim, H = params.hidden_dim;
    if (world == 1) {
        GCNHIP_CHECK(gcnhip_feat_create_aggregated(env.ctx, &feat_agg, graph, feat));
    } else {
        const std::vector<int> &fp = data->feature_index.indptr, &fi = data->feature_index.indices;
        gcnhip_graph *g_all = graph_l1;
        gcnhip_feat *x_all = feat_full;
        try {
            if (!g_all) g_all = create_rows_graph(env.ctx);
            if (!x_all)
                GCNHIP_CHECK(gcnhip_feat_create(env.ctx, &x_all, fp.data(), fi.empty() ? nullptr : fi.data(), data->feature_value.data(), N, F));
            GCNHIP_CHECK(gcnhip_feat_create_aggregated(env.ctx, &feat_agg, g_all, x_all));
        } catch (...) {
            if (g_all && g_all != graph_l1) gcnhip_graph_destroy(env.ctx, g_all);
            if (x_all && x_all != feat_full) gcnhip_feat_destroy(env.ctx, x_all);
            throw;
        }
        if (g_all != graph_l1) gcnhip_graph_destroy(env.ctx, g_all);
        if (x_all != feat_full) gcnhip_feat_destroy(env.ctx, x_all);
    }
    agg_vals = gcnhip_feat_values(feat_agg);
    auto *sm = new HipSparseMatmul(&env, &agg_vals, variables[2].get(), variables[3].get(), feat_agg, n_local, F, H, 0.f, 0);
    sm->relu_out = true;
    if (opt_.eval_fusion && !env.bf16_tables) sm->fuse_next = dynamic_cast<HipMatmul *>(modules[2]);
    eval_modules.push_back(sm);
    for (size_t i = 2; i < modules.size(); i++) eval_modules.push_back(modules[i]);
}

void HipGCN::build_eval_lane() {
    const int world = env.comm->size(), rank = env.comm->rank();
    const int N = n_local, F = params.input_dim, H = params.hidden_dim, C = params.output_dim;
    lane.reset(new EvalLane());
    EvalLane &L = *lane;
    HipSparseMatmul *lane_sm = nullptr;
    GCNHIP_CHECK(gcnhip_ctx_create(&L.env.ctx,  device_, nullptr));
    L.arena.bind(L.env.ctx);
    GCNHIP_CHECK(gcnhip_ctx_set_corun(L.env.ctx, 1));
    if (slice_floats == 32 || slice_floats == 16) GCNHIP_CHECK(gcnhip_ctx_set_option(L.env.ctx, "gs_l", slice_floats / 4));
    if (opt_.gemm >= 0) GCNHIP_CHECK(gcnhip_ctx_set_option(L.env.ctx, "gemm_bf16x3", opt_.gemm ? 2 : 0));
    L.timers.reset(new DeviceTimers(L.env.ctx));
    L.timers->enabled = timers->enabled;
    L.env.timers = L.timers.get();
    L.comm.reset(env.comm->clone_for(L.env.ctx));
    L.env.comm = L.comm.get();
    L.env.plan = &xplan;
    L.env.xbuf = &L.xbuf;
    if (world > 1) exchange_buffers_create(L.env.ctx, xplan, xbuf.max_ld_words, &L.xbuf);
    L.env.seed = env.seed;
    L.env.bf16_tables = env.bf16_tables;
    L.env.d_epoch = L.arena.alloc<uint32_t>(1);
    GCNHIP_CHECK(gcnhip_memset_async(L.env.ctx, L.env.d_epoch, 0xFF, sizeof(uint32_t)));
    L.d_result = L.arena.alloc<float>(4);
    L.d_result_i = L.arena.alloc<int32_t>(4);
    GCNHIP_CHECK(gcnhip_graph_clone(L.env.ctx, &L.graph, graph));
    if (!(flags & HIPGCN_ALL_ROWS)) add_split_rowsets(L.env.ctx, L.graph, L.split_rows);
    const ExchangePlan *xp = world > 1 ? &xplan : nullptr;
    L.H0.reset(new HipVariable()); L.H1.reset(new HipVariable()); L.Z0.reset(new HipVariable()); L.Z.reset(new HipVariable());
    if (feat_agg) {
    } else if (replicate_l1) {
        L.graph_l1 = create_rows_graph(L.env.ctx);
        apply_schedule(L.env.ctx, L.graph_l1);
        L.H0->alloc_replicated(L.env.ctx, params.num_nodes, N, part.start[rank], H, false);
    } else {
        L.H0->alloc(L.env.ctx, N, H, false, true, false, xp);
    }
    L.H1->alloc(L.env.ctx, N, H, false);
    L.Z0->alloc(L.env.ctx, N, C, false, true, false, xp);
    L.Z->alloc(L.env.ctx, N, C, false);
    const uint64_t nnz_off = (uint64_t)data->feature_index.indptr[part.start[rank]];
    eval_vals = gcnhip_feat_values(feat);
    if (feat_agg) {
        auto *sm = new HipSparseMatmul(&L.env, &agg_vals, variables[2].get(), L.H1.get(), feat_agg, N, F, H, 0.f, 0);
        sm->relu_out = true;
        lane_sm = sm;
        L.modules.push_back(sm);
    } else {
        auto *sm = new HipSparseMatmul(&L.env, &eval_vals, variables[2].get(), L.H0.get(), feat, N, F, H, 0.f, nnz_off);
        auto *gs = new HipGraphSum(&L.env, L.H0.get(), L.H1.get(), L.graph, H, 0.f, 0);
        if (factored_) gs->fwd_scaling = 2;
        if (replicate_l1) { sm->sp_full = feat_full; sm->vals_full = &full_vals; gs->fwd_graph_replicated = L.graph_l1; }
        L.modules.push_back(sm);
        L.modules.push_back(gs);
    }
    {
        auto *mm = new HipMatmul(&L.env, L.H1.get(), variables[5].get(), L.Z0.get(), N, H, C);
        if (lane_sm && opt_.eval_fusion && !L.env.bf16_tables) lane_sm->fuse_next = mm;
        L.modules.push_back(mm);
    }
    auto *gs_logits = new HipGraphSum(&L.env, L.Z0.get(), L.Z.get(), L.graph, C);
    gs_logits->fwd_out_rows = &L.scored.out_rows;
    if (factored_) gs_logits->fwd_scaling = 1;
    L.modules.push_back(gs_logits);
    L.modules.push_back(make_loss({&L.env, L.Z.get(), &L.scored, L.d_result, L.d_result_i, false, nullptr, true,
                                   gs_logits}));
    GCNHIP_CHECK(gcnhip_event_create_sync(&L.ev_weights));
    GCNHIP_CHECK(gcnhip_event_create_sync(&L.ev_done));
    GCNHIP_CHECK(gcnhip_event_create_sync(&L.ev_fork));
    GCNHIP_CHECK(gcnhip_ctx_sync(L.env.ctx));
}

void HipGCN::destroy_lane() {
    if (!lane) return;
    EvalLane &L = *lane;
    if (L.env.ctx) {
        gcnhip_ctx_sync(L.env.ctx);
        for (auto m : L.modules) delete m;
        L.modules.clear();
        L.H0.reset(); L.H1.reset(); L.Z0.reset(); L.Z.reset();
        if (L.graph) gcnhip_graph_destroy(L.env.ctx, L.graph);
        if (L.graph_l1) gcnhip_graph_destroy(L.env.ctx, L.graph_l1);
        L.arena.free_all();
        for (void *e : {L.ev_weights, L.ev_done, L.ev_fork})
            if (e) gcnhip_event_destroy(e);
        L.timers.reset();
        exchange_buffers_destroy(&L.xbuf);
        L.comm.reset();
        gcnhip_ctx_destroy(L.env.ctx);
    }
    lane.reset();
}

HipGCN::~HipGCN() { release(); }

void HipGCN::release() {
    if (!env.ctx) return;
    gcnhip_ctx_sync(env.ctx);
    destroy_lane();
    queries_.reset();
    if (!eval_modules.empty()) delete eval_modules[0];
    eval_modules.clear();
    for (auto m : modules) delete m;
    modules.clear();
    if (variables.size() == 7 && gradbuf) {
        if (variables[2]) variables[2]->grad = nullptr;
        if (variables[5]) variables[5]->grad = nullptr;
    }
    variables.clear();
    optimizer.reset();
    if (epoch_graph) { gcnhip_graph_exec_destroy(epoch_graph); epoch_graph = nullptr; }
    readback_destroy();
    env.xlane = nullptr;
    xlane.reset();
    for (gcnhip_graph *g : {graph_loc, graph_rem, graph_bwd_loc, graph_bwd_rem, graph_bwd_out, graph, graph_l1})
        if (g) gcnhip_graph_destroy(env.ctx, g);
    for (gcnhip_feat *f : {feat, feat_full, feat_agg})
        if (f) gcnhip_feat_destroy(env.ctx, f);
    arena.free_all();
    timers.reset();
    exchange_buffers_destroy(&xbuf);
    owned_comm.reset();
    gcnhip_ctx_destroy(env.ctx);
    env.ctx = nullptr;
}
```

cuda_gcn_amd/host/gcn_epochs.cpp:

```cpp
#include "gcn.h"
#include <chrono>
#include <deque>
#include <cstdio>
#include "hip_check.h"

void HipGCN::sync() {
    if (xlane) GCNHIP_CHECK(gcnhip_ctx_sync(xlane->ctx));
    GCNHIP_CHECK(gcnhip_ctx_sync(env.ctx));
    if (lane) GCNHIP_CHECK(gcnhip_ctx_sync(lane->env.ctx));
}

double HipGCN::timer_total(timer_instance t, long *count) {
    long c0 = 0, c1 = 0, c2 = 0;
    double s = timers->total(t, &c0);
    if (lane) s += lane->timers->total(t, &c1);
    if (xlane) s += xlane->timers->total(t, &c2);
    if (count) *count = c0 + c1 + c2;
    return s;
}
void HipGCN::timers_reset() {
    timers->reset();
    if (lane) lane->timers->reset();
    if (xlane) xlane->timers->reset();
}

void HipGCN::set_timers(bool on) {
    sync();
    timers->enabled = on;
    if (lane) lane->timers->enabled = on;
    if (xlane) xlane->timers->enabled = on;
}

void HipGCN::fill_scored(ScoredSplit &d, int s, gcnhip_rowset *const *rows) const {
    const bool own = rows == split_rows;
    d.truth = d_truth[s];
    d.count = split_count[s];
    d.wsum = split_wsum[s];
    d.out_rows = rows[s];
    d.out_rows_loc = own ? split_rows_loc[s] : nullptr;
    d.out_rows_rem = own ? split_rows_rem[s] : nullptr;
    d.rows = d_split_list[s];
    d.rows_n = split_local_n[s];
}

void HipGCN::set_truth(int s) { fill_scored(scored, s, split_rows); }

void HipGCN::refresh_input() {
    if (flags & HIPGCN_MODULAR)
        GCNHIP_CHECK(gcnhip_d2d_async(env.ctx, input->data, gcnhip_feat_values(feat), (size_t)gcnhip_feat_nnz(feat) * sizeof(float)));
}

void HipGCN::host_masks_for_epoch() {
    const int thr = (int)(params.dropout * MY_RAND_MAX);
    const int rank = env.comm->rank();
    const long nnz_total = data->feature_index.indptr[params.num_nodes];
    const long f0 = keep0_first;
    for (long i = 0; i < nnz_total; i++) {
        const bool keep = (int)rng.next() >= thr;
        if (i >= f0 && i < f0 + (long)h_keep0.size()) h_keep0[i - f0] = keep;
    }
    const long H = params.hidden_dim, h0 = (long)part.start[rank] * H, total = (long)params.num_nodes * H;
    for (long i = 0; i < total; i++) {
        const bool keep = (int)rng.next() >= thr;
        if (i >= h0 && i < h0 + (long)h_keep1.size()) h_keep1[i - h0] = keep;
    }
    GCNHIP_CHECK(gcnhip_h2d(env.ctx, d_keep0, h_keep0.data(), h_keep0.size()));
    GCNHIP_CHECK(gcnhip_h2d(env.ctx, d_keep1, h_keep1.data(), h_keep1.size()));
}

void HipGCN::metrics_before(HipEnv &e, int slot, const uint32_t *epoch_word) {
    if (e.comm->size() == 1 && opt_.loss_records_metrics)
        GCNHIP_CHECK(gcnhip_metrics_record_with_next_loss(e.ctx, d_ring, RING, slot, epoch_word, optimizer->d_sumsq));
}

void HipGCN::metrics_after(HipEnv &e, DeviceTimers &t, int slot, const uint32_t *epoch_word, float *result, size_t n) {
    if (e.comm->size() > 1) {
        t.start(TMR_COMM);
        e.comm->allreduce_sum(result + 4 - n, n);
        t.stop(TMR_COMM);
    }
    if (!(e.comm->size() == 1 && opt_.loss_records_metrics))
        GCNHIP_CHECK(gcnhip_metrics_record(e.ctx, d_ring, RING, slot, epoch_word, result, nullptr, optimizer->d_sumsq));
}

void HipGCN::train_begin() {
    metrics_before(env, 0, env.d_epoch);
    epochs_done++;
    refresh_input();
    if (flags & HIPGCN_HOST_MASKS) host_masks_for_epoch();
    set_truth(1);
}

void HipGCN::train_end() {
    metrics_after(env, *timers, 0, env.d_epoch, d_result, gradbuf_elems);
    if (lane && lane->pending) {
        GCNHIP_CHECK(gcnhip_stream_wait_event(env.ctx, lane->ev_done));
        lane->pending = false;
    }
    optimizer->step();
    if (lane) GCNHIP_CHECK(gcnhip_event_record(env.ctx, lane->ev_weights));
}

void HipGCN::train_epoch_async() {
    h1_from_fused_eval = false;
    train_begin();
    for (auto m : modules) m->forward(true);
    for (int i = (int)modules.size() - 1; i >= 0; i--) modules[i]->backward();
    train_end();
}

void HipGCN::lane_begin(int s) {
    EvalLane &L = *lane;
    GCNHIP_CHECK(gcnhip_stream_wait_event(L.env.ctx, L.ev_weights));
    const long want = epochs_done - 1;
    GCNHIP_CHECK(gcnhip_counter_add(L.env.ctx, L.env.d_epoch, (uint32_t)(want - L.epoch_word)));
    L.epoch_word = want;
    fill_scored(L.scored, s, L.split_rows);
    metrics_before(L.env, s == 2 ? 1 : 2, L.env.d_epoch);
}

void HipGCN::lane_end(int s) {
    EvalLane &L = *lane;
    metrics_after(L.env, *L.timers, s == 2 ? 1 : 2, L.env.d_epoch, L.d_result, 4);
    GCNHIP_CHECK(gcnhip_event_record(L.env.ctx, L.ev_done));
    L.pending = true;
}

void HipGCN::eval_on_lane(int s) {
    lane_begin(s);
    for (auto m : lane->modules) m->forward(false);
    lane_end(s);
}

void HipGCN::eval_then_train_zipped(int s) {
    lane_begin(s);
    train_begin();
    const size_t nb = lane->modules.size(), na = modules.size();
    if (env.comm->size() == 1) {
        modules[0]->forward(true);
        GCNHIP_CHECK(gcnhip_event_record(env.ctx, lane->ev_fork));
        GCNHIP_CHECK(gcnhip_stream_wait_event(lane->env.ctx, lane->ev_fork));
        for (size_t i = 0; i < nb; i++) lane->modules[i]->forward(false);
        lane_end(s);
        for (size_t i = 1; i < na; i++) modules[i]->forward(true);
        for (int i = (int)na - 1; i >= 0; i--) modules[i]->backward();
        train_end();
        return;
    }
    for (size_t i = 0; i < std::max(na, nb); i++) {
        if (i < nb) lane->modules[i]->forward(false);
        if (i < na) modules[i]->forward(true);
    }
    lane_end(s);
    for (int i = (int)na - 1; i >= 0; i--) modules[i]->backward();
    train_end();
}

void HipGCN::eval_async(int s) {
    refresh_input();
    set_truth(s);
    metrics_before(env, s == 2 ? 1 : 2, env.d_epoch_done);
    for (auto m : eval_modules.empty() ? modules : eval_modules) m->forward(false);
    h1_from_fused_eval = !eval_modules.empty() && static_cast<HipSparseMatmul *>(eval_modules[0])->hidden_not_stored;
    metrics_after(env, *timers, s == 2 ? 1 : 2, env.d_epoch_done, d_result, 4);
}

std::pair<float, float> HipGCN::read_metrics(long epoch_index, int slot) {
    float row[8];
    if (lane) GCNHIP_CHECK(gcnhip_ctx_sync(lane->env.ctx));
    const uint32_t e = (uint32_t)epoch_index;
    GCNHIP_CHECK(gcnhip_d2h(env.ctx, row, d_ring + ((size_t)(e % RING) * 4 + slot) * 8, sizeof row));
    return ring_metrics(row);
}

std::pair<float, float> HipGCN::ring_metrics(const float *row) const {
    const float l2 = params.weight_decay * row[4] / 2;
    if (opt_.multilabel)
        return {row[0] / row[1] + l2, row[3] > 0.f ? row[2] / row[3] : 0.f};
    if (!opt_.class_weights.empty())
        return {row[0] / row[1] + l2, (float)row[2] / (int)row[3]};
    const float loss = row[0] / (int)row[1];
    const float acc = (float)row[2] / (int)row[3];
    return {loss + l2, acc};
}

std::pair<float, float> HipGCN::train_epoch() {
    train_epoch_async();
    return read_metrics(epochs_done - 1, 0);
}

std::pair<float, float> HipGCN::eval(int s) {
    eval_async(s);
    return read_metrics(epochs_done - 1, s == 2 ? 1 : 2);
}

bool HipGCN::enqueue_epoch_replay() {
    const bool graph_ok = env.comm->size() == 1 && !lane && !timers->enabled && !(flags & (HIPGCN_HOST_MASKS | HIPGCN_NO_GRAPH));
    if (!(graph_ok && epochs_done >= 1 && optimizer->can_replay(1))) return false;
    if (!epoch_graph) {
        const long epochs_before = epochs_done;
        const int steps_before = optimizer->steps();
        GCNHIP_CHECK(gcnhip_capture_begin(env.ctx));
        try {
            train_epoch_async();
            eval_async(2);
        } catch (...) {
            void *broken = nullptr;
            gcnhip_capture_end(env.ctx, &broken);
            if (broken) gcnhip_graph_exec_destroy(broken);
            epochs_done = epochs_before;
            optimizer->note_replayed(steps_before - optimizer->steps());
            throw;
        }
        GCNHIP_CHECK(gcnhip_capture_end(env.ctx, &epoch_graph));
        epochs_done = epochs_before;
        optimizer->note_replayed(steps_before - optimizer->steps());
    }
    GCNHIP_CHECK(gcnhip_graph_launch(env.ctx, epoch_graph));
    epochs_done++;
    optimizer->note_replayed(1);
    return true;
}

void HipGCN::enqueue_epoch(bool first, bool last) {
    if (zipped()) {
        if (first) train_epoch_async();
        if (last) eval_on_lane(2); else eval_then_train_zipped(2);
// ... 182 lines not shown
```

cuda_gcn_amd/host/module.cpp:

```cpp
#include "module.h"
#include <algorithm>
#include "hip_check.h"

HipMatmul::HipMatmul(HipEnv *env, HipVariable *a, HipVariable *b, HipVariable *c, int m, int n, int p, float s)
    : env(env), a(a), b(b), c(c), m(m), n(n), p(p), fused_bwd_scale(s) {}

bool HipMatmul::fused_eval_forward(gcnhip_feat *sp, const float *vals, HipVariable *w1, int p1) {
    if (p1 != n) return false;
    const int rc = gcnhip_spmm_fwd_relu_matmul(env->ctx, sp, vals, w1->data, w1->ld, p1, b->data, b->ld, p, c->data, c->ld);
    if (rc == GCNHIP_NOT_AVAILABLE) return false;
    GCNHIP_CHECK(rc);
    skip_forward_once = true;
    return true;
}

void HipMatmul::forward(bool) {
    if (skip_forward_once) { skip_forward_once = false; return; }
    env->timers->start(TMR_MATMUL_FW);
    GCNHIP_CHECK(gcnhip_matmul_fwd(env->ctx, a->data, a->ld, b->data, b->ld, c->data, c->ld, m, n, p));
    env->timers->stop(TMR_MATMUL_FW);
}

void HipMatmul::backward() {
    env->timers->start(TMR_MATMUL_BW);
    if (pos_bits_full && env->xlane) {
        void *ev = env->xlane->begin(*env->plan, c->full_grad, c->ld);
        GCNHIP_CHECK(gcnhip_matmul_bwd(env->ctx, a->data, a->ld, b->data, b->ld, c->grad, c->ld,
                                       nullptr, a->ld, b->grad, b->ld, m, n, p));
        const int own = env->plan->own_offset;
        rebuild_da(own, m);
        env->xlane->wait(ev);
        if (env->pos_bits_ready) { env->xlane->wait(env->pos_bits_ready); env->pos_bits_ready = nullptr; }
        rebuild_da(0, own);
        rebuild_da(own + m, all_rows - own - m);
    } else if (pos_bits_full) {
        GCNHIP_CHECK(gcnhip_matmul_bwd(env->ctx, a->data, a->ld, b->data, b->ld, c->grad, c->ld,
                                       nullptr, a->ld, b->grad, b->ld, m, n, p));
        env->timers->stop(TMR_MATMUL_BW);
        env->timers->start(TMR_COMM);
        env->comm->exchange_rows(*env->plan, *env->xbuf, c->full_grad, c->ld);
        env->timers->stop(TMR_COMM);
        env->timers->start(TMR_MATMUL_BW);
        rebuild_da(0, all_rows);
    } else if (fused_bwd_scale > 0.f)
        GCNHIP_CHECK(gcnhip_matmul_bwd_ex(env->ctx, a->data, a->ld, b->data, b->ld, c->grad, c->ld, a->grad, a->ld, b->grad, b->ld, m, n, p,
                                          fused_bwd_scale, mask_bits, mask_bits ? mask_wpr : 0, da_row_scale));
    else
        GCNHIP_CHECK(gcnhip_matmul_bwd(env->ctx, a->data, a->ld, b->data, b->ld, c->grad, c->ld,
                                       a->grad, a->ld, b->grad, b->ld, m, n, p));
    env->timers->stop(TMR_MATMUL_BW);
}

void HipMatmul::rebuild_da(int first, int rows) {
    if (rows <= 0) return;
    GCNHIP_CHECK(gcnhip_matmul_bwd_ex(env->ctx, nullptr, 0, b->data, b->ld, c->full_grad + (size_t)first * c->ld, c->ld,
                                      a->full_grad + (size_t)first * a->ld, a->ld, nullptr, 0, rows, n, p, fused_bwd_scale,
                                      pos_bits_full + (size_t)first * wpr, wpr, da_row_scale_full ? da_row_scale_full + first : nullptr));
}

HipSparseMatmul::HipSparseMatmul(HipEnv *env, const float *const *vals, HipVariable *b, HipVariable *c, gcnhip_feat *sp,
                                 int m, int n, int p, float fd, uint64_t off)
    : env(env), vals(vals), b(b), c(c), sp(sp), m(m), n(n), p(p), fused_dropout(fd), nnz_offset(off) {}

void HipSparseMatmul::forward(bool training) {
    last_training = training;
    if (training) fwd_decisions_valid = fused_dropout > 0.f && !sp_full && !relu_out && gcnhip_feat_is_dense(sp);
    env->timers->start(TMR_SPMATMUL_FW);
    const float pd = training ? fused_dropout : 0.f;
    hidden_not_stored = false;
    if (relu_out) {
        if (training) throw GcnHipFailure(-1, "HipSparseMatmul: the ReLU epilogue is an evaluation-only form");
        if (fuse_next && fuse_next->fused_eval_forward(sp, *vals, b, p)) hidden_not_stored = true;
        else GCNHIP_CHECK(gcnhip_spmm_fwd_relu(env->ctx, sp, *vals, b->data, b->ld, c->data, c->ld, p));
    } else if (sp_full)
        GCNHIP_CHECK(gcnhip_spmm_fwd(env->ctx, sp_full, *vals_full, b->data, b->ld, c->full, c->ld, p, pd,
                                     env->seed ^ KEY_INPUT_DROPOUT, env->d_epoch, 0,
                                     pd > 0.f ? env->keep_input : nullptr));
    else
        GCNHIP_CHECK(gcnhip_spmm_fwd(env->ctx, sp, *vals, b->data, b->ld, c->data, c->ld, p, pd,
                                     env->seed ^ KEY_INPUT_DROPOUT, env->d_epoch, nnz_offset,
                                     pd > 0.f ? env->keep_input : nullptr));
    env->timers->stop(TMR_SPMATMUL_FW);
}

void HipSparseMatmul::forward_stored() {
    if (!relu_out) throw GcnHipFailure(-1, "HipSparseMatmul::forward_stored: an evaluation-only form");
    GCNHIP_CHECK(gcnhip_spmm_fwd_relu(env->ctx, sp, *vals, b->data, b->ld, c->data, c->ld, p));
    hidden_not_stored = false;
}

void HipSparseMatmul::backward() {
    env->timers->start(TMR_SPMATMUL_BW);
    const float pd = last_training ? fused_dropout : 0.f;
    int rps = 0, n_splits = 0;
    GCNHIP_CHECK(gcnhip_spmm_bwd_plan(env->ctx, sp, p, &rps, &n_splits));
    if (n_splits > 0 && pd > 0.f && fwd_decisions_valid) {
        GCNHIP_CHECK(gcnhip_spmm_bwd_part(env->ctx, sp, *vals, c->grad, c->ld, p, pd, env->seed ^ KEY_INPUT_DROPOUT, env->d_epoch,
                                          nnz_offset, env->keep_input_bwd, 0, n_splits, 0));
        GCNHIP_CHECK(gcnhip_spmm_bwd_finish(env->ctx, sp, b->grad, b->ld, p));
    } else {
        GCNHIP_CHECK(gcnhip_spmm_bwd(env->ctx, sp, *vals, c->grad, c->ld, b->grad, b->ld, p, pd,
                                     env->seed ^ KEY_INPUT_DROPOUT, env->d_epoch, nnz_offset,
                                     pd > 0.f ? env->keep_input_bwd : nullptr));
    }
    env->timers->stop(TMR_SPMATMUL_BW);
}

HipGraphSum::HipGraphSum(HipEnv *env, HipVariable *in, HipVariable *out, gcnhip_graph *graph, int dim, float frd, uint64_t off)
    : env(env), in(in), out(out), graph(graph), dim(dim), fused_relu_dropout(frd), elem_offset(off) {}

HipGraphSum::~HipGraphSum() { if (bf_table) gcnhip_free(env->ctx, bf_table); }

size_t HipGraphSum::full_rows(const HipVariable *v, bool grad) {
    const float *full = grad ? v->full_grad : v->full;
    return full ? v->full_elems / v->ld : (size_t)v->rows;
}

uint16_t *HipGraphSum::table() {
    if (!bf_table) {
        ld_bf = dim <= 8 ? 8 : (dim <= 16 ? 16 : (dim <= 32 ? 32 : (dim + 63) / 64 * 64));
        bf_rows = std::max(full_rows(in, false), full_rows(out, true));
        void *p;
        GCNHIP_CHECK(gcnhip_malloc(env->ctx, &p, bf_rows * ld_bf * sizeof(uint16_t)));
        GCNHIP_CHECK(gcnhip_memset_async(env->ctx, p, 0, bf_rows * ld_bf * sizeof(uint16_t)));
        bf_table = (uint16_t *)p;
    }
    return bf_table;
}

void HipGraphSum::forward(bool training) {
    gcnhip_graph *graph = this->graph;
    const int world = env->comm->size();
    const gcnhip_rowset *out_rows = fwd_out_rows ? *fwd_out_rows : nullptr;
    const bool replicated = in->replicated && fwd_graph_replicated;
    if (replicated) graph = fwd_graph_replicated;
    bool bits_written = false;
    if (env->bf16_tables) {
        uint16_t *tab = table();
        env->timers->start(TMR_GRAPHSUM_FW);
        if (replicated) {
            GCNHIP_CHECK(gcnhip_f32_to_bf16(env->ctx, in->full, in->ld, tab, ld_bf, (int64_t)full_rows(in, false), dim));
        } else {
            const size_t own = world > 1 ? (size_t)env->plan->own_offset : 0;
            GCNHIP_CHECK(gcnhip_f32_to_bf16(env->ctx, in->data, in->ld, tab + own * ld_bf, ld_bf, in->rows, dim));
            if (world > 1) {
                env->timers->start(TMR_COMM);
                env->comm->exchange_rows(*env->plan, *env->xbuf, reinterpret_cast<float *>(tab), ld_bf / 2);
                env->timers->stop(TMR_COMM);
            }
        }
        if (dim > 64) env->timers->start(TMR_GRAPHSUM_WIDE);
        const bool fused = fused_relu_dropout >= 0.f;
        if (predict)
            GCNHIP_CHECK(gcnhip_graphsum_predict(env->ctx, graph, predict->rows, nullptr, tab, ld_bf, nullptr, 0, dim, 0, predict->pred,
                                                 predict->prob, predict->logp, predict->ld_logp));
        else
            GCNHIP_CHECK(gcnhip_graphsum_bf16(env->ctx, graph, tab, ld_bf, redirect ? redirect->data : out->data, redirect ? redirect->ld : out->ld, dim,
                                              nullptr, redirect ? redirect->rows : out_rows, fused ? 1 : 0, training ? 1 : 0,
                                              fused ? fused_relu_dropout : 0.f, env->seed ^ KEY_HIDDEN_DROPOUT, env->d_epoch, elem_offset,
                                              training ? env->keep_hidden : nullptr));
        if (dim > 64) env->timers->stop(TMR_GRAPHSUM_WIDE);
        env->timers->stop(TMR_GRAPHSUM_FW);
    } else if (env->xlane && !replicated && world > 1 && !predict && !redirect) {
        void *ev = env->xlane->begin(*env->plan, in->full, in->ld);
// ... 52 lines not shown
    }
    if (pos_bits_full && training) {
        uint32_t *mine = pos_bits_full + (size_t)env->plan->own_offset * wpr;
        if (!bits_written) GCNHIP_CHECK(gcnhip_pack_positive(env->ctx, out->data, out->ld, out->rows, dim, mine, wpr));
        if (env->xlane) {
            if (env->pos_bits_ready) env->xlane->wait(env->pos_bits_ready);
            env->pos_bits_ready = env->xlane->begin(*env->plan, reinterpret_cast<float *>(pos_bits_full), wpr);
        } else {
            env->timers->start(TMR_COMM);
            env->comm->exchange_rows(*env->plan, *env->xbuf, reinterpret_cast<float *>(pos_bits_full), wpr);
            env->timers->stop(TMR_COMM);
        }
    }
}

void HipGraphSum::backward() {
    const int world = env->comm->size();
    const uint32_t *row_bits = bwd_row_bits && !bwd_graph ? *bwd_row_bits : nullptr;
    const gcnhip_graph *graph = bwd_graph ? bwd_graph : this->graph;
    if (env->bf16_tables) {
        uint16_t *tab = table();
        env->timers->start(TMR_GRAPHSUM_BW);
        if (world > 1 && out_grad_complete) {
            GCNHIP_CHECK(gcnhip_f32_to_bf16(env->ctx, out->full_grad, out->ld, tab, ld_bf, (int64_t)full_rows(out, true), dim));
        } else {
            const size_t own = world > 1 ? (size_t)env->plan->own_offset : 0;
            GCNHIP_CHECK(gcnhip_f32_to_bf16(env->ctx, out->grad, out->ld, tab + own * ld_bf, ld_bf, out->rows, dim));
            if (world > 1) {
                env->timers->start(TMR_COMM);
                env->comm->exchange_rows(*env->plan, *env->xbuf, reinterpret_cast<float *>(tab), ld_bf / 2);
                env->timers->stop(TMR_COMM);
            }
        }
        if (dim > 64) env->timers->start(TMR_GRAPHSUM_WIDE);
        GCNHIP_CHECK(gcnhip_graphsum_bf16(env->ctx, graph, tab, ld_bf, in->grad, in->ld, dim, row_bits, nullptr, 0, 0, 0.f, 0, nullptr, 0, nullptr));
        if (dim > 64) env->timers->stop(TMR_GRAPHSUM_WIDE);
        env->timers->stop(TMR_GRAPHSUM_BW);
        return;
    }
    if (world > 1 && !out_grad_complete && env->xlane) {
        const gcnhip_graph *loc = bwd_split_loc ? bwd_split_loc : split_loc, *rem = bwd_split_rem ? bwd_split_rem : split_rem;
        const uint32_t *bits = bwd_split_loc ? nullptr : row_bits;
        void *ev = env->xlane->begin(*env->plan, out->full_grad, out->ld);
        env->timers->start(TMR_GRAPHSUM_BW);
        if (dim > 64) env->timers->start(TMR_GRAPHSUM_WIDE);
        gcnhip_gs_opts o = {};
        o.in_row_bits = bits; o.scaling = bwd_scaling;
        if (loc) GCNHIP_CHECK(gcnhip_graphsum_ex(env->ctx, loc, &o, out->full_grad, out->ld, in->grad, in->ld, dim));
        env->xlane->wait(ev);
        o.accumulate = 1;
        if (rem) GCNHIP_CHECK(gcnhip_graphsum_ex(env->ctx, rem, &o, out->full_grad, out->ld, in->grad, in->ld, dim));
        if (dim > 64) env->timers->stop(TMR_GRAPHSUM_WIDE);
        env->timers->stop(TMR_GRAPHSUM_BW);
        return;
    }
    if (world > 1 && !out_grad_complete) {
        env->timers->start(TMR_COMM);
        env->comm->exchange_rows(*env->plan, *env->xbuf, out->full_grad, out->ld);
        env->timers->stop(TMR_COMM);
    }
    const float *src = out->full_grad ? out->full_grad : out->grad;
    env->timers->start(TMR_GRAPHSUM_BW);
    if (dim > 64) env->timers->start(TMR_GRAPHSUM_WIDE);
    gcnhip_gs_opts o = {};
    o.in_row_bits = row_bits; o.scaling = bwd_scaling;
    GCNHIP_CHECK(gcnhip_graphsum_ex(env->ctx, graph, &o, src, out->ld, in->grad, in->ld, dim));
    if (dim > 64) env->timers->stop(TMR_GRAPHSUM_WIDE);
    env->timers->stop(TMR_GRAPHSUM_BW);
}

HipCrossEntropyLoss::HipCrossEntropyLoss(HipEnv *env, HipVariable *logits, int32_t *const *truth, const int *count,
                                         float *d_result, int32_t *d_result_i, int num_classes, bool shift)
    : env(env), logits(logits), truth(truth), count(count), d_result(d_result), d_result_i(d_result_i),
      num_classes(num_classes), shift_in_place(shift) {}


bool HipCrossEntropyLoss::epilogue_opts(bool training, gcnhip_gs_loss *o) const {
    if (!row_terms || !rows_list || !*rows_list || *count <= 0 || num_classes > 64 || shift_in_place || d_weight) return false;
    o->truth = *truth; o->grad = logits->grad; o->ld_grad = logits->ld; o->training = training ? 1 : 0; o->count = *count;
    o->grad_row_scale = grad_row_scale; o->row_terms = row_terms;
    return true;
}

void HipCrossEntropyLoss::forward(bool training) {
    env->timers->start(TMR_LOSS_FW);
    if (d_weight)
        GCNHIP_CHECK(gcnhip_wxent_fwd_rows(env->ctx, logits->data, logits->ld, logits->grad, logits->ld, *truth, *rows_list, rows_n ? *rows_n : 0,
                                           num_classes, training && *count > 0 ? 1 : 0, *count > 0 ? *count : 1, shift_in_place ? 1 : 0,
                                           d_result, d_result_i, grad_row_scale, d_weight, *weight_sum));
    else if (terms_fresh) {
        terms_fresh = false;
        GCNHIP_CHECK(gcnhip_xent_from_row_terms(env->ctx, row_terms, *truth, *rows_list, *rows_n, d_result, d_result_i));
    } else if (rows_list && *rows_list && *count > 0)
        GCNHIP_CHECK(gcnhip_xent_fwd_rows_scaled(env->ctx, logits->data, logits->ld, logits->grad, logits->ld, *truth, *rows_list, *rows_n,
                                                 num_classes, training ? 1 : 0, *count, shift_in_place ? 1 : 0, d_result, d_result_i,
                                                 grad_row_scale));
    else
    GCNHIP_CHECK(gcnhip_xent_fwd(env->ctx, logits->data, logits->ld, logits->grad, logits->ld, *truth, logits->rows,
                                 num_classes, training ? 1 : 0, *count, shift_in_place ? 1 : 0, d_result, d_result_i));
    env->timers->stop(TMR_LOSS_FW);
}

HipBCELoss::HipBCELoss(HipEnv *env, HipVariable *logits, const uint32_t *truth, int wpr, const int *count,
                       float *d_result, int32_t *d_result_i, int num_classes)
    : env(env), logits(logits), truth(truth), wpr(wpr), count(count), d_result(d_result), d_result_i(d_result_i),
      num_classes(num_classes) {}

void HipBCELoss::forward(bool training) {
    env->timers->start(TMR_LOSS_FW);
    const int n = rows_n ? *rows_n : 0;
    if (d_pos_weight)
        GCNHIP_CHECK(gcnhip_wbce_fwd_rows(env->ctx, logits->data, logits->ld, logits->grad, logits->ld, truth, wpr, *rows_list, n, num_classes,
                                          training && *count > 0 ? 1 : 0, *count, grad_row_scale, d_result, d_result_i, d_pos_weight));
    else
    GCNHIP_CHECK(gcnhip_bce_fwd_rows(env->ctx, logits->data, logits->ld, logits->grad, logits->ld, truth, wpr, *rows_list, n, num_classes,
                                     training && *count > 0 ? 1 : 0, *count, grad_row_scale, d_result, d_result_i));
    env->timers->stop(TMR_LOSS_FW);
}

HipReLU::HipReLU(HipEnv *env, HipVariable *in) : env(env), in(in), mask(nullptr) {
    void *p;
    GCNHIP_CHECK(gcnhip_malloc(env->ctx, &p, (size_t)in->rows * in->cols));
    mask = (uint8_t *)p;
}
HipReLU::~HipReLU() { gcnhip_free(env->ctx, mask); }
void HipReLU::forward(bool training) {
    env->timers->start(TMR_RELU_FW);
    GCNHIP_CHECK(gcnhip_relu_fwd_2d(env->ctx, in->data, in->ld, in->rows, in->cols, mask, training ? 1 : 0));
    env->timers->stop(TMR_RELU_FW);
}
void HipReLU::backward() {
    env->timers->start(TMR_RELU_BW);
    GCNHIP_CHECK(gcnhip_relu_bwd_2d(env->ctx, in->grad, in->ld, in->rows, in->cols, mask));
    env->timers->stop(TMR_RELU_BW);
}

HipDropout::HipDropout(HipEnv *env, HipVariable *in, float p, uint64_t key_tweak, uint64_t elem_offset, const uint8_t *const *keep_in)
    : env(env), in(in), mask(nullptr), p(p), key_tweak(key_tweak), elem_offset(elem_offset), keep_in(keep_in) {
    if (in->grad) {
        void *q;
        GCNHIP_CHECK(gcnhip_malloc(env->ctx, &q, (size_t)in->rows * in->cols * sizeof(int32_t)));
        mask = (int32_t *)q;
    }
}
HipDropout::~HipDropout() { if (mask) gcnhip_free(env->ctx, mask); }
void HipDropout::forward(bool training) {
    if (!training) return;
    env->timers->start(TMR_DROPOUT_FW);
    GCNHIP_CHECK(gcnhip_dropout_fwd_2d(env->ctx, in->data, in->ld, in->rows, in->cols, mask, p, env->seed ^ key_tweak,
                                       env->d_epoch, elem_offset, *keep_in));
    env->timers->stop(TMR_DROPOUT_FW);
}
void HipDropout::backward() {
    if (!mask) return;
    env->timers->start(TMR_DROPOUT_BW);
    GCNHIP_CHECK(gcnhip_dropout_bwd_2d(env->ctx, in->grad, in->ld, in->rows, in->cols, mask, p));
    env->timers->stop(TMR_DROPOUT_BW);
}
```

cuda_gcn_amd/host/module.h:

```cpp
#pragma once
#include <vector>
#include <cstdint>
#include "comm.h"
#include "gcnhip_driver.h"
#include "timer.h"
#include "variable.h"

struct HipEnv {
    gcnhip_ctx *ctx = nullptr;
    Comm *comm = nullptr;
    const ExchangePlan *plan = nullptr;
    ExchangeBuffers *xbuf = nullptr;
    DeviceTimers *timers = nullptr;
    uint64_t seed = 0;
    uint32_t *d_epoch = nullptr;
    uint32_t *d_epoch_done = nullptr;
    const uint8_t *keep_input = nullptr;
    const uint8_t *keep_input_bwd = nullptr;
    const uint8_t *keep_hidden = nullptr;
    bool bf16_tables = false;
    ExchangeLane *xlane = nullptr;
    void *pos_bits_ready = nullptr;
};

class Module {
public:
    virtual void forward(bool) = 0;
    virtual void backward() = 0;
    virtual ~Module() {}
};

class HipMatmul : public Module {
    HipEnv *env;
    HipVariable *a, *b, *c;
    int m, n, p;
    float fused_bwd_scale;
public:
    const uint32_t *pos_bits_full = nullptr;
    int wpr = 0, all_rows = 0;
    const uint32_t *mask_bits = nullptr;
    int mask_wpr = 0;
    const float *da_row_scale = nullptr, *da_row_scale_full = nullptr;
    HipMatmul(HipEnv *env, HipVariable *a, HipVariable *b, HipVariable *c, int m, int n, int p, float fused_bwd_scale = 0.f);
    bool fused_eval_forward(gcnhip_feat *sp, const float *vals, HipVariable *w1, int p1);
private:
    bool skip_forward_once = false;
    void rebuild_da(int first_row, int n_rows);
public:
    void forward(bool) override;
    void backward() override;
};

class HipSparseMatmul : public Module {
    HipEnv *env;
    const float *const *vals;
    HipVariable *b, *c;
    gcnhip_feat *sp;
    int m, n, p;
    float fused_dropout;
    uint64_t nnz_offset;
    bool last_training = false;
    bool fwd_decisions_valid = false;
public:
    gcnhip_feat *sp_full = nullptr;
    const float *const *vals_full = nullptr;
    bool relu_out = false;
    HipMatmul *fuse_next = nullptr;
    bool hidden_not_stored = false;
    void forward_stored();
    HipSparseMatmul(HipEnv *env, const float *const *vals, HipVariable *b, HipVariable *c, gcnhip_feat *sp,
                    int m, int n, int p, float fused_dropout, uint64_t nnz_offset);
    void forward(bool) override;
    void backward() override;
};

class HipCrossEntropyLoss;
class HipGraphSum : public Module {
    HipEnv *env;
    HipVariable *in, *out;
    gcnhip_graph *graph;
    int dim;
    float fused_relu_dropout;
    uint64_t elem_offset;
public:
    HipCrossEntropyLoss *loss = nullptr;
    gcnhip_graph *fwd_graph_replicated = nullptr;
    uint32_t *pos_bits_full = nullptr;
    int wpr = 0;
    bool out_grad_complete = false;
    uint32_t *mask_bits_out = nullptr;
    const uint32_t *const *bwd_row_bits = nullptr;
    const gcnhip_graph *bwd_graph = nullptr;
    gcnhip_rowset *const *fwd_out_rows = nullptr;
    const gcnhip_graph *split_loc = nullptr, *split_rem = nullptr;
    const gcnhip_graph *bwd_split_loc = nullptr, *bwd_split_rem = nullptr;
    gcnhip_rowset *const *fwd_out_rows_loc = nullptr, *const *fwd_out_rows_rem = nullptr;
    int fwd_scaling = 0, bwd_scaling = 0;
    struct Prediction {
        const gcnhip_rowset *rows = nullptr;
        int32_t *pred = nullptr;
        float *prob = nullptr, *logp = nullptr;
        int ld_logp = 0;
    };
    const Prediction *predict = nullptr;
    struct Redirect {
        float *data = nullptr;
        int ld = 0;
        const gcnhip_rowset *rows = nullptr;
    };
    const Redirect *redirect = nullptr;
    HipGraphSum(HipEnv *env, HipVariable *in, HipVariable *out, gcnhip_graph *graph, int dim,
                float fused_relu_dropout = -1.f, uint64_t elem_offset = 0);
    ~HipGraphSum() override;
    void forward(bool) override;
    void backward() override;
private:
    uint16_t *bf_table = nullptr;
    int ld_bf = 0;
    size_t bf_rows = 0;
    uint16_t *table();
    static size_t full_rows(const HipVariable *v, bool grad);
};

class HipCrossEntropyLoss : public Module {
    HipEnv *env;
    HipVariable *logits;
    int32_t *const *truth;
    const int *count;
    float *d_result;
    int32_t *d_result_i;
    int num_classes;
    bool shift_in_place;
public:
    int32_t *const *rows_list = nullptr;
    const int *rows_n = nullptr;
    const float *grad_row_scale = nullptr;
    float *row_terms = nullptr;
    bool terms_fresh = false;
    bool epilogue_opts(bool training, gcnhip_gs_loss *o) const;
    const float *d_weight = nullptr;
    const float *weight_sum = nullptr;
    HipCrossEntropyLoss(HipEnv *env, HipVariable *logits, int32_t *const *truth, const int *count,
                        float *d_result, int32_t *d_result_i, int num_classes, bool shift_in_place);
    void forward(bool) override;
    void backward() override {}
};

class HipBCELoss : public Module {
    HipEnv *env;
    HipVariable *logits;
    const uint32_t *truth;
    int wpr;
    const int *count;
    float *d_result;
    int32_t *d_result_i;
    int num_classes;
public:
    int32_t *const *rows_list = nullptr;
    const int *rows_n = nullptr;
    const float *grad_row_scale = nullptr;
    const float *d_pos_weight = nullptr;
    HipBCELoss(HipEnv *env, HipVariable *logits, const uint32_t *truth, int wpr, const int *count,
               float *d_result, int32_t *d_result_i, int num_classes);
    void forward(bool) override;
    void backward() override {}
};

class HipReLU : public Module {
    HipEnv *env;
    HipVariable *in;
    uint8_t *mask;
public:
    HipReLU(HipEnv *env, HipVariable *in);
    ~HipReLU() override;
    void forward(bool) override;
    void backward() override;
};

class HipDropout : public Module {
    HipEnv *env;
    HipVariable *in;
    int32_t *mask;
    float p;
    uint64_t key_tweak, elem_offset;
    const uint8_t *const *keep_in;
public:
    HipDropout(HipEnv *env, HipVariable *in, float p, uint64_t key_tweak, uint64_t elem_offset, const uint8_t *const *keep_in);
    ~HipDropout() override;
    void forward(bool) override;
    void backward() override;
};

constexpr uint64_t KEY_INPUT_DROPOUT = 0x9E3779B97F4A7C15ull;
constexpr uint64_t KEY_HIDDEN_DROPOUT = 0xD1B54A32D192ED03ull;
```

cuda_gcn_amd/ops.py:

```python
from __future__ import annotations

import ctypes as C

import numpy as np

from . import _lib


class GsOpts(C.Structure):
    _fields_ = [("rows", C.c_void_p), ("in_row_bits", C.c_void_p), ("accumulate", C.c_int), ("relu_dropout", C.c_int), ("training", C.c_int),
                ("p", C.c_float), ("seed", C.c_uint64), ("d_epoch", C.c_void_p), ("elem_offset", C.c_uint64), ("keep_mask", C.c_void_p),
                ("pos_bits", C.c_void_p), ("words_per_row", C.c_int), ("scaling", C.c_int), ("loss", C.c_void_p)]


class GsLoss(C.Structure):
    _fields_ = [("truth", C.c_void_p), ("grad", C.c_void_p), ("ld_grad", C.c_int), ("training", C.c_int), ("count", C.c_int),
                ("grad_row_scale", C.c_void_p), ("row_terms", C.c_void_p)]


class GcnHipError(RuntimeError):
    pass


def _ck(lib, code, what):
# ... 600 lines not shown
        return out.download()[:, :dim]

    def graphsum_relu_dropout_bits(self, g, x, training, p, seed=0, epoch=0, elem_offset=0, keep_mask=None, ld=None):
        x = np.asarray(x, np.float32)
        dim = x.shape[1]
        ld = ld or dim
        wpr = (dim + 31) // 32
        xin = self.padded(x, ld)
        out = self.buf(np.full((g.n_rows, ld), np.nan, np.float32))
        bits = self.buf(np.full((g.n_rows, wpr), 0xDEADBEEF, np.uint32))
        g.reserve(dim)
        ep = self.buf(np.array([epoch], np.uint32))
        km = self.buf(np.ascontiguousarray(keep_mask, np.uint8)) if keep_mask is not None else None
        _ck(self.lib, self.lib.gcnhip_graphsum_relu_dropout_bits(self.ctx, g.h, xin.ptr, ld, out.ptr, ld, dim, int(training), p, seed, ep.ptr,
                                                                  elem_offset, km.ptr if km else None, bits.ptr, wpr), "graphsum_relu_dropout_bits")
        return out.download()[:, :dim], bits.download()

    def matmul_bwd_fused_bits(self, a, b, dc, scale, bits):
        a, b, dc = (np.asarray(t, np.float32) for t in (a, b, dc))
        m, n = a.shape
        p = b.shape[1]
        ldp = (p + 3) // 4 * 4
        ab, bb, dcb = self.buf(a), self.padded(b, ldp), self.padded(dc, ldp)
        bt = self.buf(np.ascontiguousarray(bits, np.uint32))
        da = self.buf(np.full((m, n), np.nan, np.float32))
        db = self.buf(np.full((n, ldp), np.nan, np.float32))
        _ck(self.lib, self.lib.gcnhip_matmul_bwd_fused_bits(self.ctx, ab.ptr, n, bb.ptr, ldp, dcb.ptr, ldp, da.ptr, n, db.ptr, ldp, m, n, p, scale,
                                                             bt.ptr, bits.shape[1]), "gcnhip_matmul_bwd_fused_bits")
        return da.download(), db.download()[:, :p]

    def matmul_bwd_ex(self, a, b, dc, scale, bits, rowscale=None, ldp=None, p=None):
        a, b, dc = (np.asarray(t, np.float32) for t in (a, b, dc))
        m, n = a.shape
        p = p or b.shape[1]
        ldp = ldp or (p + 3) // 4 * 4
        ab, bb, dcb = self.buf(a), self.padded(b, ldp), self.padded(dc, ldp)
        bt = self.buf(np.ascontiguousarray(bits, np.uint32))
        rs = self.buf(np.ascontiguousarray(rowscale, np.float32)) if rowscale is not None else None
        da = self.buf(np.full((m, n), np.nan, np.float32))
        db = self.buf(np.full((n, ldp), np.nan, np.float32))
        _ck(self.lib, self.lib.gcnhip_matmul_bwd_ex(self.ctx, ab.ptr, n, bb.ptr, ldp, dcb.ptr, ldp, da.ptr, n, db.ptr, ldp, m, n, p, scale,
                                                     bt.ptr, bits.shape[1], rs.ptr if rs else None), "gcnhip_matmul_bwd_ex")
        return da.download(), db.download()[:, :p]

    SLACK_ROWS = 2

    def _operand(self, arr, ld, shift=0, fill=np.nan):
        arr = np.asarray(arr, np.float32)
        rows, cols = arr.shape
        flat = np.full(shift + (rows + self.SLACK_ROWS) * ld + 4, fill, np.float32)
        table = flat[shift:shift + rows * ld].reshape(rows, ld)
        table[:, :cols] = arr
        b = self.buf(flat)
        return b, b.ptr + 4 * shift, rows * ld

    @staticmethod
    def _table(buf, shift, rows, ld, cols, whole):
        flat = buf.download()
        table = flat[shift:shift + rows * ld].reshape(rows, ld)
        return table if whole else table[:, :cols].copy()

    def _vals(self, f, vals, shift):
        if vals is None:
            return None, f.values_ptr
        b, ptr, _ = self._operand(np.ascontiguousarray(vals, np.float32).reshape(1, -1), max(int(np.size(vals)), 1), shift)
        return b, ptr

    def spmm_fwd(self, f: "Feat", w, p_drop=0.0, seed=0, epoch=0, nnz_offset=0, keep_mask=None, vals=None, ld_w=None, ld_out=None,
                 whole=False, fill=np.nan, shift=None):
        w = np.asarray(w, np.float32)
        p = w.shape[1]
        ld_w = ld_w or p
        ld_out = ld_out or p
        sh = shift or {}
        wb, wptr, _ = self._operand(w, ld_w, sh.get("w", 0))
        out, optr, _ = self._operand(np.zeros((f.n_rows, 0), np.float32), ld_out, sh.get("out", 0), fill)
        ep = self.buf(np.array([epoch], np.uint32))
        km = self.buf(np.ascontiguousarray(keep_mask, np.uint8)) if keep_mask is not None else None
        vb, vptr = self._vals(f, vals, sh.get("vals", 0))
        _ck(self.lib, self.lib.gcnhip_spmm_fwd(self.ctx, f.h, vptr, wptr, ld_w, optr, ld_out, p, p_drop, seed, ep.ptr,
                                                nnz_offset, km.ptr if km else None), "gcnhip_spmm_fwd")
        return self._table(out, sh.get("out", 0), f.n_rows, ld_out, p, whole)

    def spmm_fwd_relu(self, f: "Feat", w, ld_w=None, ld_out=None, vals=None, whole=False, fill=np.nan, shift=None):
        w = np.asarray(w, np.float32)
        p = w.shape[1]
        ld_w, ld_out = ld_w or p, ld_out or p
        sh = shift or {}
        wb, wptr, _ = self._operand(w, ld_w, sh.get("w", 0))
        out, optr, _ = self._operand(np.zeros((f.n_rows, 0), np.float32), ld_out, sh.get("out", 0), fill)
        vb, vptr = self._vals(f, vals, sh.get("vals", 0))
        _ck(self.lib, self.lib.gcnhip_spmm_fwd_relu(self.ctx, f.h, vptr, wptr, ld_w, optr, ld_out, p), "gcnhip_spmm_fwd_relu")
        return self._table(out, sh.get("out", 0), f.n_rows, ld_out, p, whole)

    def spmm_fwd_relu_matmul(self, f: "Feat", w, w2, ld_z=None, vals=None, ld_w=None, ld_w2=None, whole=False, fill=np.nan, shift=None):
        w, w2 = np.asarray(w, np.float32), np.asarray(w2, np.float32)
        p, p2 = w.shape[1], w2.shape[1]
        ld_z = ld_z or (p2 + 3) // 4 * 4
        ld_w, ld_w2 = ld_w or p, ld_w2 or ld_z
        sh = shift or {}
        wb, wptr, _ = self._operand(w, ld_w, sh.get("w", 0))
        w2b, w2ptr, _ = self._operand(w2, ld_w2, sh.get("w2", 0))
        z, zptr, _ = self._operand(np.zeros((f.n_rows, 0), np.float32), ld_z, sh.get("out", 0), fill)
        vb, vptr = self._vals(f, vals, sh.get("vals", 0))
        rc = self.lib.gcnhip_spmm_fwd_relu_matmul(self.ctx, f.h, vptr, wptr, ld_w, p, w2ptr, ld_w2, p2, zptr, ld_z)
        if rc == -2:
            return None
        _ck(self.lib, rc, "gcnhip_spmm_fwd_relu_matmul")
        return self._table(z, sh.get("out", 0), f.n_rows, ld_z, p2, whole)

    def spmm_bwd(self, f: "Feat", dout, p_drop=0.0, seed=0, epoch=0, nnz_offset=0, keep_mask=None, vals=None, ld_dout=None, ld_dw=None,
                 whole=False, fill=np.nan, shift=None):
        dout = np.asarray(dout, np.float32)
        p = dout.shape[1]
        ld_dout = ld_dout or p
        ld_dw = ld_dw or p
        sh = shift or {}
        db, dptr, _ = self._operand(dout, ld_dout, sh.get("dout", 0))
        dw, wptr, _ = self._operand(np.zeros((f.n_cols, 0), np.float32), ld_dw, sh.get("out", 0), fill)
        ep = self.buf(np.array([epoch], np.uint32))
        km = self.buf(np.ascontiguousarray(keep_mask, np.uint8)) if keep_mask is not None else None
        vb, vptr = self._vals(f, vals, sh.get("vals", 0))
        _ck(self.lib, self.lib.gcnhip_spmm_bwd(self.ctx, f.h, vptr, dptr, ld_dout, wptr, ld_dw, p, p_drop, seed, ep.ptr,
                                                nnz_offset, km.ptr if km else None), "gcnhip_spmm_bwd")
        return self._table(dw, sh.get("out", 0), f.n_cols, ld_dw, p, whole)

    def spmm_bwd_plan(self, f: "Feat", p):
        rps, ns = C.c_int(), C.c_int()
        _ck(self.lib, self.lib.gcnhip_spmm_bwd_plan(self.ctx, f.h, p, C.byref(rps), C.byref(ns)), "gcnhip_spmm_bwd_plan")
        return rps.value, ns.value

    def spmm_bwd_parts(self, f: "Feat", dout, cuts, p_drop=0.0, seed=0, epoch=0, nnz_offset=0, order=None, make_first=True, keep_mask=None,
                       vals=None, ld_dout=None, ld_dw=None, whole=False, fill=np.nan, shift=None):
        dout = np.asarray(dout, np.float32)
        p = dout.shape[1]
        ld_dout, ld_dw = ld_dout or p, ld_dw or p
        sh = shift or {}
        db, dptr, _ = self._operand(dout, ld_dout, sh.get("dout", 0))
        dw, wptr, _ = self._operand(np.zeros((f.n_cols, 0), np.float32), ld_dw, sh.get("out", 0), fill)
        ep = self.buf(np.array([epoch], np.uint32))
        km = self.buf(np.ascontiguousarray(keep_mask, np.uint8)) if keep_mask is not None else None
        vb, vptr = self._vals(f, vals, sh.get("vals", 0))
        ranges = list(zip(cuts[:-1], cuts[1:]))
        for k, i in enumerate(order if order is not None else range(len(ranges))):
            _ck(self.lib, self.lib.gcnhip_spmm_bwd_part(self.ctx, f.h, vptr, dptr, ld_dout, p, p_drop, seed, ep.ptr, nnz_offset,
                                                         km.ptr if km else None, ranges[i][0], ranges[i][1],
                                                         1 if (k == 0 and make_first) else 0), "gcnhip_spmm_bwd_part")
        _ck(self.lib, self.lib.gcnhip_spmm_bwd_finish(self.ctx, f.h, wptr, ld_dw, p), "gcnhip_spmm_bwd_finish")
        return self._table(dw, sh.get("out", 0), f.n_cols, ld_dw, p, whole)

    def matmul_fwd(self, a, b, lda=None, ldb=None, ldc=None):
        a, b = np.asarray(a, np.float32), np.asarray(b, np.float32)
        m, n = a.shape
        p = b.shape[1]
        lda, ldb, ldc = lda or n, ldb or p, ldc or p
        ab, bb = self.padded(a, lda), self.padded(b, ldb)
        cb = self.buf(np.full((m, ldc), np.nan, np.float32))
        _ck(self.lib, self.lib.gcnhip_matmul_fwd(self.ctx, ab.ptr, lda, bb.ptr, ldb, cb.ptr, ldc, m, n, p), "gcnhip_matmul_fwd")
        return cb.download()[:, :p]

    def matmul_bwd(self, a, b, dc, lda=None, ldb=None, lddc=None, fused_scale=None):
        a, b, dc = (np.asarray(t, np.float32) for t in (a, b, dc))
        m, n = a.shape
        p = b.shape[1]
        lda, ldb, lddc = lda or n, ldb or p, lddc or p
        ab, bb, dcb = self.padded(a, lda), self.padded(b, ldb), self.padded(dc, lddc)
# ... 481 lines not shown
```

include/gcnhip_driver.h:

```cpp
#ifndef GCNHIP_DRIVER_H
#define GCNHIP_DRIVER_H
#include "gcnhip.h"
#ifdef __cplusplus
extern "C" {
#endif

typedef struct gcnhip_rowset gcnhip_rowset;

int gcnhip_ctx_set_corun(gcnhip_ctx *ctx, int on);
int gcnhip_host_alloc(void **ptr, size_t bytes);
int gcnhip_host_free(void *ptr);
int gcnhip_d2h_async(gcnhip_ctx *ctx, void *dst_pinned, const void *src, size_t bytes);
int gcnhip_graph_create_grouped(gcnhip_ctx *ctx, gcnhip_graph **g, const int *h_indptr, const int *h_indices,
                                int n_rows, int n_cols, const int *h_col_deg, const int *h_row_group);
int gcnhip_graph_set_schedule(gcnhip_ctx *ctx, gcnhip_graph *g, int mode, const int *h_row_group, int n_groups);
int gcnhip_graphsum_rowmask(gcnhip_ctx *ctx, const gcnhip_graph *g, const float *in, int ld_in,
                            float *out, int ld_out, int dim, const uint32_t *in_row_bits);
int gcnhip_graphsum_masked(gcnhip_ctx *ctx, const gcnhip_graph *g, const float *in, int ld_in,
                           float *out, int ld_out, int dim, const uint32_t *in_row_bits, const uint32_t *out_row_bits);
int gcnhip_graph_add_rowset(gcnhip_ctx *ctx, gcnhip_graph *g, const uint32_t *h_row_bits, gcnhip_rowset **rows);
int gcnhip_rowset_size(const gcnhip_rowset *rows, int *n_tasks);
int gcnhip_graphsum_rowset(gcnhip_ctx *ctx, const gcnhip_graph *g, const gcnhip_rowset *rows, const float *in, int ld_in,
                           float *out, int ld_out, int dim, const uint32_t *in_row_bits);
int gcnhip_graph_create_restricted(gcnhip_ctx *ctx, gcnhip_graph **out, const gcnhip_graph *parent, const uint32_t *h_col_bits);
// ... 20 lines not shown
    const uint32_t *d_epoch;
    uint64_t elem_offset;
    const uint8_t *keep_mask;
    uint32_t *pos_bits;
    int words_per_row;
    int scaling;
    const struct gcnhip_gs_loss *loss;
} gcnhip_gs_opts;
typedef struct gcnhip_gs_loss {
    const int32_t *truth;
    float *grad; int ld_grad;
    int training, count;
    const float *grad_row_scale;
    float *row_terms;
} gcnhip_gs_loss;
int gcnhip_graphsum_ex(gcnhip_ctx *ctx, const gcnhip_graph *g, const gcnhip_gs_opts *opts, const float *in, int ld_in,
                       float *out, int ld_out, int dim);
int gcnhip_graphsum_predict(gcnhip_ctx *ctx, const gcnhip_graph *g, const gcnhip_rowset *rows, const float *in, const uint16_t *in_bf16,
                            int ld_in, float *out, int ld_out, int dim, int scaling, int32_t *pred, float *prob, float *logp, int ld_logp);
int gcnhip_graphsum_blend(gcnhip_ctx *ctx, const gcnhip_graph *g, const float *in, int ld_in, const float *base, int ld_base,
                          float *out, int ld_out, int dim, float alpha, float beta, float lo, float hi, int32_t *pred);
int gcnhip_cs_error_rows(gcnhip_ctx *ctx, const float *logp, int ld_logp, const int32_t *truth, int n_table, const int32_t *d_rows,
                         int n_listed, int num_classes, float *e, int ld_e, float *d_sigma);
int gcnhip_cs_correct_rows(gcnhip_ctx *ctx, const float *logp, int ld_logp, const float *e_hat, int ld_e, const int32_t *truth, int n_table,
                           int num_classes, const float *d_sigma, float *g0, int ld_g);
int gcnhip_calib_nll_rows(gcnhip_ctx *ctx, const float *logp, int ld, const int32_t *truth, int n_table, const int32_t *d_rows, int n,
                          int num_classes, float beta, double *d_out);
int gcnhip_calib_bins_rows(gcnhip_ctx *ctx, const float *logp, int ld, const int32_t *truth, int n_table, const int32_t *d_rows, int n,
                           int num_classes, float beta, int bins, int32_t *d_count, int32_t *d_correct, double *d_conf_sum);
int gcnhip_calib_scale_rows(gcnhip_ctx *ctx, const float *logp, int ld, int n_table, const int32_t *d_rows, int n, int num_classes, float beta,
                            float *out_logp, int ld_out, float *d_prob);
int gcnhip_conformal_scores(gcnhip_ctx *ctx, const float *logp, int ld, int n_table, const int32_t *d_rows, int n, int num_classes, float beta,
                            int method, float lam, int k_reg, float *out, int ld_out);
int gcnhip_conformal_true_scores(gcnhip_ctx *ctx, const float *table, int ld, const int32_t *truth, int n_table, const int32_t *d_rows, int n,
                                 int num_classes, float *d_score);
int gcnhip_conformal_sets_rows(gcnhip_ctx *ctx, const float *table, int ld, int n_table, const int32_t *d_rows, int n, int num_classes,
                               const float *d_thresh, const int32_t *truth, uint32_t *d_bits, int32_t *d_size, int32_t *d_counts);
#define GCNHIP_SORT_TILE 4096
#define GCNHIP_RANK_STATS_BLOCKS 32
int gcnhip_sort_tile(void);
int gcnhip_rank_keys(gcnhip_ctx *ctx, const float *table, int ld, int n_table, const int32_t *d_rows, int n, int c0, int c1, int num_classes,
                     const int32_t *truth, const uint32_t *truth_bits, int words_per_row, uint32_t *pos_keys, uint32_t *neg_keys, int64_t stride,
                     int32_t *d_pos, int32_t *d_neg, int32_t *d_invalid, int32_t *d_unlabelled);
int gcnhip_sort_segments_u32(gcnhip_ctx *ctx, uint32_t *keys, uint32_t *scratch, int n, int segments, int64_t stride);
int gcnhip_rank_stats(gcnhip_ctx *ctx, const uint32_t *pos_keys, const uint32_t *neg_keys, int64_t stride, int n, int segments, const int32_t *d_pos,
                      const int32_t *d_neg, void *d_work, int64_t *d_u2, double *d_ap_sum);
int gcnhip_embed_inv_norms(gcnhip_ctx *ctx, const float *table, int ld, int n_table, int dim, float *inv_norm);
int gcnhip_topk_plan(int n_table, int nq, int k, int chunk_rows, int *chunk_rows_used, int *n_chunks, size_t *scratch_bytes,
                     size_t *scratch_bytes_min);
int gcnhip_topk_rows(gcnhip_ctx *ctx, const float *table, int ld, int n_table, int dim, const float *inv_norm, const int32_t *row_id,
                     const int32_t *q_rows, int nq, int k, int exclude_self, int chunk_rows, void *scratch, size_t scratch_bytes,
                     int launches, int32_t *out_id, float *out_score);
int gcnhip_pair_scores(gcnhip_ctx *ctx, const float *table, int ld, int n_table, int dim, const float *inv_norm, const int32_t *src,
                       const int32_t *dst, int n_pairs, float *out);
int gcnhip_embed_rows(gcnhip_ctx *ctx, const float *table, int ld, int n_table, int dim, const float *inv_norm, const int32_t *d_rows,
                      int n, float *out, int ld_out);
int gcnhip_explain_hops(gcnhip_ctx *ctx, const gcnhip_graph *g, const int32_t *q_row, const int32_t *q_class, int nq, const float *h1,
                        int ld_h1, int h, const float *w2, int ld_w2, int num_classes, int scaling, float *logit, float *hidden,
                        int ld_out, const int32_t *nbr_ptr, int32_t *nbr_row, float *nbr_val, int64_t nbr_capacity);
int gcnhip_explain_features_agg(gcnhip_ctx *ctx, const gcnhip_graph *g, const int32_t *q_row, const int32_t *q_class, int nq,
                                const float *h1, int ld_h1, int h, const float *w2, int ld_w2, int num_classes, const float *w1,
                                int ld_w1, int n_features, const float *s, int ld_s, int scaling, float *feat, int ld_f);
int gcnhip_explain_features_walk(gcnhip_ctx *ctx, const gcnhip_graph *g, const gcnhip_feat *x, const int32_t *q_row,
                                 const int32_t *q_class, int nq, const float *h1, int ld_h1, int h, const float *w2, int ld_w2,
                                 int num_classes, const float *w1, int ld_w1, int scaling, float *feat, int ld_f);
int gcnhip_explain_abs_colsum(gcnhip_ctx *ctx, const float *feat, int ld_f, const int32_t *q_class, int nq, int n_features,
                              int num_classes, double *acc, int32_t *count);
int gcnhip_graph_remove_rowset(gcnhip_ctx *ctx, gcnhip_graph *g, gcnhip_rowset *rows);
int gcnhip_graph_scales(const gcnhip_graph *g, const float **d_dinv_row, const float **d_dinv2_row,
                        const float **d_dinv_col, const float **d_dinv2_col);
int gcnhip_feat_scale_rows(gcnhip_ctx *ctx, gcnhip_feat *f, const float *d_row_scale);

int gcnhip_feat_create_aggregated(gcnhip_ctx *ctx, gcnhip_feat **f, gcnhip_graph *g, const gcnhip_feat *x);
int gcnhip_spmm_fwd_relu(gcnhip_ctx *ctx, const gcnhip_feat *f, const float *vals, const float *w, int ld_w,
                         float *out, int ld_out, int p);
#define GCNHIP_NOT_AVAILABLE (-2)
int gcnhip_spmm_fwd_relu_matmul(gcnhip_ctx *ctx, const gcnhip_feat *f, const float *vals, const float *w, int ld_w, int p,
                                const float *w2, int ld_w2, int p2, float *z0, int ld_z0);
int gcnhip_spmm_bwd_plan(const gcnhip_ctx *ctx, const gcnhip_feat *f, int p, int *rows_per_split, int *n_splits);
int gcnhip_spmm_bwd_part(gcnhip_ctx *ctx, const gcnhip_feat *f, const float *vals, const float *dout, int ld_dout, int p,
                         float p_drop, uint64_t seed, const uint32_t *d_epoch, uint64_t nnz_offset, const uint8_t *keep_mask,
                         int split_begin, int split_end, int make_decisions);
int gcnhip_spmm_bwd_finish(gcnhip_ctx *ctx, const gcnhip_feat *f, float *dw, int ld_dw, int p);

int gcnhip_f32_to_bf16(gcnhip_ctx *ctx, const float *src, int ld_src, uint16_t *dst, int ld_dst, int64_t rows, int dim);
int gcnhip_graphsum_bf16(gcnhip_ctx *ctx, const gcnhip_graph *g, const uint16_t *in_bf16, int ld_in,
                         float *out, int ld_out, int dim, const uint32_t *in_row_bits, const gcnhip_rowset *out_rows,
                         int relu_dropout, int training, float p, uint64_t seed, const uint32_t *d_epoch,
                         uint64_t elem_offset, const uint8_t *keep_mask);

int gcnhip_matmul_bwd_fused(gcnhip_ctx *ctx, const float *a, int lda, const float *b, int ldb,
                            const float *dc, int lddc, float *da, int ldda, float *db, int lddb,
                            int m, int n, int p, float relu_dropout_scale);
int gcnhip_matmul_bwd_fused_bits(gcnhip_ctx *ctx, const float *a, int lda, const float *b, int ldb,
                                 const float *dc, int lddc, float *da, int ldda, float *db, int lddb,
                                 int m, int n, int p, float relu_dropout_scale, const uint32_t *pos_bits, int words_per_row);

int gcnhip_matmul_bwd_ex(gcnhip_ctx *ctx, const float *a, int lda, const float *b, int ldb,
                         const float *dc, int lddc, float *da, int ldda, float *db, int lddb,
                         int m, int n, int p, float relu_dropout_scale, const uint32_t *pos_bits, int words_per_row,
                         const float *d_da_row_scale);

int gcnhip_pack_positive(gcnhip_ctx *ctx, const float *h, int ld, int n_rows, int dim, uint32_t *bits, int words_per_row);
int gcnhip_matmul_bwd_da_bits(gcnhip_ctx *ctx, const float *b, int ldb, const float *dc, int lddc,
                              float *da, int ldda, int m, int n, int p,
                              const uint32_t *h_pos_bits, int words_per_row, float scale);

int gcnhip_gather_rows(gcnhip_ctx *ctx, const float *src, int ld_words, const int *d_rows, int n, float *dst);

int gcnhip_relu_dropout_bwd(gcnhip_ctx *ctx, float *grad, int ld_grad, const float *h, int ld_h,
                            int n_rows, int dim, float scale);

int gcnhip_xent_fwd_rows(gcnhip_ctx *ctx, float *logits, int ld, float *grad, int ld_grad,
                         const int32_t *truth, const int32_t *d_rows, int n_listed, int num_classes, int training,
                         int count, int shift_in_place, float *d_result, int32_t *d_result_i);
int gcnhip_xent_fwd_rows_scaled(gcnhip_ctx *ctx, float *logits, int ld, float *grad, int ld_grad,
                                const int32_t *truth, const int32_t *d_rows, int n_listed, int num_classes, int training,
                                int count, int shift_in_place, float *d_result, int32_t *d_result_i, const float *d_grad_row_scale);
int gcnhip_xent_from_row_terms(gcnhip_ctx *ctx, const float *d_row_terms, const int32_t *truth, const int32_t *d_rows, int n_listed,
                               float *d_result, int32_t *d_result_i);
int gcnhip_bce_fwd_rows(gcnhip_ctx *ctx, const float *logits, int ld, float *grad, int ld_grad,
                        const uint32_t *truth_bits, int words_per_row, const int32_t *d_rows, int n_listed,
                        int num_classes, int training, int count, const float *d_grad_row_scale,
                        float *d_result, int32_t *d_result_i);
int gcnhip_bce_predict_rows(gcnhip_ctx *ctx, const float *logits, int ld, const int32_t *d_rows, int n_rows, int num_classes,
                            uint32_t *bits, int words_per_row, float *prob, int ld_prob);
int gcnhip_wxent_fwd_rows(gcnhip_ctx *ctx, float *logits, int ld, float *grad, int ld_grad,
                          const int32_t *truth, const int32_t *d_rows, int n_listed, int num_classes, int training,
                          int count, int shift_in_place, float *d_result, int32_t *d_result_i, const float *d_grad_row_scale,
                          const float *d_class_weight, float weight_sum);
int gcnhip_wbce_fwd_rows(gcnhip_ctx *ctx, const float *logits, int ld, float *grad, int ld_grad,
                         const uint32_t *truth_bits, int words_per_row, const int32_t *d_rows, int n_listed,
                         int num_classes, int training, int count, const float *d_grad_row_scale,
                         float *d_result, int32_t *d_result_i, const float *d_pos_weight);
int gcnhip_confusion_rows(gcnhip_ctx *ctx, const int32_t *pred, const int32_t *truth, int n_table, const int32_t *d_rows, int n,
                          int num_classes, int32_t *counts, int32_t *out_of_range);
int gcnhip_bce_class_counts_rows(gcnhip_ctx *ctx, const float *logits, int ld, const uint32_t *truth_bits, int words_per_row,
                                 const int32_t *d_rows, int n, int num_classes, int32_t *counts);
int gcnhip_adam_step_advance(gcnhip_ctx *ctx, const gcnhip_adam_var *vars, int n_vars, float step_size,
                             const float *d_step_sizes, const uint32_t *d_epoch,
                             float beta1, float beta2, float eps, float weight_decay, float *d_sumsq,
                             uint32_t *d_epoch_counter, uint32_t *d_epoch_done);

int gcnhip_counter_add(gcnhip_ctx *ctx, uint32_t *d_counter, uint32_t inc);
int gcnhip_metrics_record(gcnhip_ctx *ctx, float *d_ring, int capacity, int slot_in_row,
                          const uint32_t *d_epoch, const float *d_result, const int32_t *d_result_i,
                          const float *d_sumsq);
int gcnhip_metrics_record_with_next_loss(gcnhip_ctx *ctx, float *d_ring, int capacity, int slot_in_row,
                                         const uint32_t *d_epoch, const float *d_sumsq);

int gcnhip_capture_begin(gcnhip_ctx *ctx);
int gcnhip_capture_end(gcnhip_ctx *ctx, void **graph_exec);
int gcnhip_graph_launch(gcnhip_ctx *ctx, void *graph_exec);
int gcnhip_graph_exec_destroy(void *graph_exec);

#ifdef __cplusplus
}
#endif
#endif
```

Baseline: 348.2.

## Draw next epoch's dropout keep-bits and loss sums on the side lane stream

Adds a side-stream kernel launch that precomputes the next epoch's input-dropout keep bitmask (epoch+1) into a second buffer. At the start of the next epoch that buffer is swapped in, so the forward SpMM can skip drawing the bits itself. Training loss/metric reduction is also deferred onto the eval lane stream so it overlaps with backward. This adds event synchronisation and an extra buffer. It also relies on the epoch counter advancing by exactly one for the precomputed bits to be correct.

Measured after the change: 349.3 (median of 6 runs). No clear change (+0.3%).

```diff
diff --git a/cuda_gcn_amd/_lib.py b/cuda_gcn_amd/_lib.py
--- a/cuda_gcn_amd/_lib.py
+++ b/cuda_gcn_amd/_lib.py
@@ -139,6 +139,9 @@
     "gcnhip_spmm_bwd_plan": (I, [P, P, I, C.POINTER(I), C.POINTER(I)]),
     "gcnhip_spmm_bwd_part": (I, [P, P, P, P, I, I, F, U64, P, U64, P, I, I, I]),
     "gcnhip_spmm_bwd_finish": (I, [P, P, P, I, I]),
+    "gcnhip_feat_draw_keep_words_ahead": (I, [P, P, F, U64, P, C.c_uint32, U64]),
+    "gcnhip_feat_take_keep_words": (I, [P]),
+    "gcnhip_spmm_fwd_drawn": (I, [P, P, P, P, I, P, I, I, F]),
     "gcnhip_matmul_fwd": (I, [P, P, I, P, I, P, I, I, I, I]),
     "gcnhip_matmul_bwd": (I, [P, P, I, P, I, P, I, P, I, P, I, I, I, I]),
     "gcnhip_matmul_bwd_fused": (I, [P, P, I, P, I, P, I, P, I, P, I, I, I, I, F]),
diff --git a/cuda_gcn_amd/csrc/common.h b/cuda_gcn_amd/csrc/common.h
--- a/cuda_gcn_amd/csrc/common.h
+++ b/cuda_gcn_amd/csrc/common.h
@@ -102,6 +102,8 @@
     DevBuf<float> csc_val;
     DevBuf<uint32_t> keep_bits;
     int keep_layout = 0;
+    DevBuf<uint32_t> keep_bits_ahead;
+    size_t keep_words = 0;
     DevBuf<int4> bwd_tasks;
     int n_bwd_tasks = 0, bwd_nw = 0;
     DevBuf<int4> bwd_split;
diff --git a/cuda_gcn_amd/csrc/dense_bf16x3.h b/cuda_gcn_amd/csrc/dense_bf16x3.h
--- a/cuda_gcn_amd/csrc/dense_bf16x3.h
+++ b/cuda_gcn_amd/csrc/dense_bf16x3.h
@@ -50,6 +50,7 @@
 struct BxBitsArgs {
     uint32_t *bits; int m, K, n_chunks, R;
     int thr; uint64_t seed; const uint32_t *d_epoch; uint64_t off; const uint8_t *keep_mask;
+    uint32_t epoch_bias;
 };
 constexpr int BX_BITS_LDS_WORDS = 4096;
 __device__ inline void dropbits_cm_body(int wg, int tid, const BxBitsArgs &b, uint32_t *lds) {
@@ -60,7 +61,7 @@
     if (!b.keep_mask) {
         const uint64_t bit1 = b.off + (uint64_t)rb * b.K + 64;
         const int n_blk = (int)((bit1 >> 7) - q0) + 1;
-        const uint32_t epoch = b.d_epoch ? *b.d_epoch : 0u;
+        const uint32_t epoch = (b.d_epoch ? *b.d_epoch : 0u) + b.epoch_bias;
         for (int blk = tid; blk < n_blk; blk += 256) {
             const uint64_t c = q0 + (uint64_t)blk;
             uint32_t ge[4] = {0xFFFFFFFFu, 0xFFFFFFFFu, 0xFFFFFFFFu, 0xFFFFFFFFu};
diff --git a/cuda_gcn_amd/csrc/feat.hip b/cuda_gcn_amd/csrc/feat.hip
--- a/cuda_gcn_amd/csrc/feat.hip
+++ b/cuda_gcn_amd/csrc/feat.hip
@@ -45,7 +45,8 @@
     if (nnz) GCNHIP_TRY(hipMemcpy(f->values, h_values, (size_t)nnz * sizeof(float), hipMemcpyHostToDevice));
     {
         const size_t words_cm = dense ? (size_t)n_rows * ((n_cols + 31) / 32) : 0;
-        GCNHIP_TRY(f->keep_bits.alloc(std::max((size_t)(nnz / 32), words_cm) + 32));
+        f->keep_words = std::max((size_t)(nnz / 32), words_cm) + 32;
+        GCNHIP_TRY(f->keep_bits.alloc(f->keep_words));
     }
     if (dense && n_cols % 128 != 0 && n_cols >= 64) {
         f->ld_pad = (n_cols + 127) / 128 * 128;
diff --git a/cuda_gcn_amd/csrc/spmm.hip b/cuda_gcn_amd/csrc/spmm.hip
--- a/cuda_gcn_amd/csrc/spmm.hip
+++ b/cuda_gcn_amd/csrc/spmm.hip
@@ -154,7 +154,7 @@
     BxBitsArgs b;
     b.bits = f->keep_bits; b.m = f->n_rows; b.K = f->n_cols; b.n_chunks = (f->n_cols + 31) / 32;
     b.R = std::max(1, std::min(128, (BX_BITS_LDS_WORDS - 12) * 32 / std::max(1, f->n_cols)));
-    b.thr = d.thr; b.seed = d.seed; b.d_epoch = d.d_epoch; b.off = d.off; b.keep_mask = d.keep_mask;
+    b.thr = d.thr; b.seed = d.seed; b.d_epoch = d.d_epoch; b.off = d.off; b.keep_mask = d.keep_mask; b.epoch_bias = 0;
     return b;
 }
 static inline bool keep_bits_cm_fit(const gcnhip_feat *f) { return f->dense && f->keep_bits && f->n_cols / 32 + 16 <= BX_BITS_LDS_WORDS; }
@@ -199,13 +199,15 @@
     return fast && t.p == 128 && c->opt.gemm_bf16x3 && !d.on && aligned16(t.x) && zf.p2 >= 1 && zf.p2 <= 64 && zf.ld_z0 % 4 == 0 &&
            zf.ld_z0 >= zf.p2 && zf.ld_w2 >= zf.p2 && aligned16(zf.z0) && (size_t)n_chunks * 2 * BX_BH_BYTES + BX_W2_BYTES <= c->wpack_bytes;
 }
-static int dense_fwd_bf16x3(gcnhip_ctx *c, const gcnhip_feat *f, const Tile128Args &t, const DropSpec &d, bool fast, const Z0Fuse *zf) {
+static int dense_fwd_bf16x3(gcnhip_ctx *c, const gcnhip_feat *f, const Tile128Args &t, const DropSpec &d, bool fast, const Z0Fuse *zf,
+                            bool drawn = false) {
     if (zf && !dense_fwd_bf16x3_z0_fits(c, t, d, fast, *zf)) return GCNHIP_NOT_AVAILABLE;
-    if (!dense_fwd_bf16x3_fits(c, f, t, d, fast, zf != nullptr)) return NOT_MINE;
+    if (!dense_fwd_bf16x3_fits(c, f, t, d, fast, zf != nullptr)) return drawn ? GCNHIP_NOT_AVAILABLE : NOT_MINE;
+    if (drawn && !(d.on && f->keep_layout == 1)) return GCNHIP_NOT_AVAILABLE;
     const int n_chunks = (t.K + PG_BK - 1) / PG_BK, n_hs = 2 * n_chunks;
     uint4 *wp3 = reinterpret_cast<uint4 *>((float *)c->wpack);
     uint4 *w2img = wp3 + (size_t)n_hs * (BX_BH_BYTES / 16);
-    if (d.on) {
+    if (d.on && !drawn) {
         const BxBitsArgs kb = keep_bits_cm_args(f, d);
         const int n_bits_wgs = ceil_div(kb.m, kb.R);
         const_cast<gcnhip_feat *>(f)->keep_layout = 1;
@@ -275,10 +277,11 @@
 
 static int spmm_fwd_impl(gcnhip_ctx *c, const gcnhip_feat *f, const float *vals, const float *w, int ld_w,
                          float *out, int ld_out, int p, float p_drop, uint64_t seed, const uint32_t *d_epoch,
-                         uint64_t nnz_offset, const uint8_t *keep_mask, int relu, const Z0Fuse *zf = nullptr) {
+                         uint64_t nnz_offset, const uint8_t *keep_mask, int relu, const Z0Fuse *zf = nullptr, bool drawn = false) {
     if (!c || !f || !vals || !w || (!out && !zf) || p <= 0 || ld_w < p || (out && ld_out < p)) return -1;
     if (!(p_drop >= 0.f && p_drop < 1.f)) return -1;
     if (zf && !(f->dense && p == 128)) return GCNHIP_NOT_AVAILABLE;
+    if (drawn && !(f->dense && p > 64)) return GCNHIP_NOT_AVAILABLE;
     if (f->n_rows == 0) return 0;
     const DropSpec d = make_drop(p_drop, seed, d_epoch, nnz_offset, keep_mask);
     if (f->dense && p > 64) {
@@ -289,6 +292,7 @@
         if (vals == f->values && f->values_pad) { t.x = f->values_pad; t.ldx = f->ld_pad; vx = 4; }
         t.m = f->n_rows; t.K = f->n_cols; t.p = p; t.bits = d.on ? f->keep_bits : nullptr; t.scale = d.scale; t.rows_per_split = 0; t.relu = relu;
         const bool fast = vx == 4 && t.ldx % 4 == 0 && (t.K + 31) / 32 * 32 <= t.ldx && ld_w % 4 == 0 && p % T_BN == 0 && aligned16(w);
+        if (drawn) return dense_fwd_bf16x3(c, f, t, d, fast, nullptr, true);
         int rc = dense_fwd_bf16x3(c, f, t, d, fast, zf);
         if (rc == NOT_MINE) rc = dense_fwd_persist(c, f, t, d, fast);
         if (rc == NOT_MINE) rc = dense_fwd_tiles(c, f, t, d, fast, vx);
@@ -377,6 +381,35 @@
     if (!w2 || !z0 || p2 <= 0) return -1;
     const Z0Fuse zf = {w2, ld_w2, p2, z0, ld_z0};
     return spmm_fwd_impl(c, f, vals, w, ld_w, nullptr, 0, p, 0.f, 0, nullptr, 0, nullptr, 1, &zf);
+}
+
+int gcnhip_spmm_fwd_drawn(gcnhip_ctx *c, const gcnhip_feat *f, const float *vals, const float *w, int ld_w,
+                          float *out, int ld_out, int p, float p_drop) {
+    if (!(p_drop > 0.f)) return -1;
+    return spmm_fwd_impl(c, f, vals, w, ld_w, out, ld_out, p, p_drop, 0, nullptr, 0, nullptr, 0, nullptr, true);
+}
+
+int gcnhip_feat_draw_keep_words_ahead(gcnhip_ctx *c, gcnhip_feat *f, float p_drop, uint64_t seed, const uint32_t *d_epoch,
+                                      uint32_t epoch_bias, uint64_t nnz_offset) {
+    if (!c || !f || !d_epoch || !(p_drop > 0.f && p_drop < 1.f)) return -1;
+    if (!keep_bits_cm_fit(f) || !c->opt.gemm_bf16x3 || f->n_rows == 0) return GCNHIP_NOT_AVAILABLE;
+    if (!f->keep_bits_ahead) {
+        GCNHIP_TRY(hipSetDevice(c->device));
+        GCNHIP_TRY(hipStreamSynchronize(c->stream));
+        GCNHIP_TRY(f->keep_bits_ahead.alloc(f->keep_words));
+    }
+    BxBitsArgs b = keep_bits_cm_args(f, make_drop(p_drop, seed, d_epoch, nnz_offset, nullptr));
+    b.bits = f->keep_bits_ahead; b.epoch_bias = epoch_bias;
+    dropbits_cm_kernel<<<ceil_div(b.m, b.R), 256, 0, c->stream>>>(b);
+    GCNHIP_LAUNCH_CHECK();
+    return 0;
+}
+
+int gcnhip_feat_take_keep_words(gcnhip_feat *f) {
+    if (!f || !f->keep_bits || !f->keep_bits_ahead) return -1;
+    std::swap(f->keep_bits, f->keep_bits_ahead);
+    f->keep_layout = 1;
+    return 0;
 }
 
 static bool dense_bwd_plan(const gcnhip_ctx *c, const gcnhip_feat *f, int p, int *rps_out, int *S_out) {
diff --git a/cuda_gcn_amd/host/gcn.h b/cuda_gcn_amd/host/gcn.h
--- a/cuda_gcn_amd/host/gcn.h
+++ b/cuda_gcn_amd/host/gcn.h
@@ -252,6 +252,7 @@
         ScoredSplit scored;
         void *ev_weights = nullptr, *ev_done = nullptr;
         void *ev_fork = nullptr;
+        void *ev_terms = nullptr;
         bool pending = false;
         long epoch_word = -1;
     };
@@ -266,6 +267,12 @@
     void eval_then_train_zipped(int current_split);
     void train_begin();
     void train_end();
+    HipCrossEntropyLoss *train_ce = nullptr;
+    bool train_sums_deferred = false;
+    void train_sums_on_lane();
+    HipSparseMatmul *train_sm = nullptr;
+    long keep_drawn_for = -1;
+    void draw_keep_words_ahead();
     void refresh_input();
     void metrics_before(HipEnv &e, int slot, const uint32_t *epoch_word);
     void metrics_after(HipEnv &e, DeviceTimers &t, int slot, const uint32_t *epoch_word, float *result, size_t n);
diff --git a/cuda_gcn_amd/host/gcn_build.cpp b/cuda_gcn_amd/host/gcn_build.cpp
--- a/cuda_gcn_amd/host/gcn_build.cpp
+++ b/cuda_gcn_amd/host/gcn_build.cpp
@@ -385,6 +385,7 @@
         auto *gs = new HipGraphSum(&env, H0, H1, graph, H, p, hid_off);
         auto *mm = new HipMatmul(&env, H1, W2, Z0, N, H, C, scale);
         if (replicate_l1) { sm->sp_full = feat_full; sm->vals_full = &full_vals; gs->fwd_graph_replicated = graph_l1; }
+        else train_sm = sm;
         wire_overlap(gs, false);
         if (factored_) {
             const float *dinv_row = nullptr, *dinv2_row = nullptr, *dinv2_col = nullptr;
@@ -421,6 +422,7 @@
         const float *dinv = nullptr;
         if (factored_) GCNHIP_CHECK(gcnhip_graph_scales(graph, &dinv, nullptr, nullptr, nullptr));
         modules.push_back(make_loss({&env, Z, &scored, d_result, d_result_i, false, dinv, true, gs_logits}));
+        train_ce = dynamic_cast<HipCrossEntropyLoss *>(modules.back());
     }
 }
 
@@ -537,6 +539,7 @@
     GCNHIP_CHECK(gcnhip_event_create_sync(&L.ev_weights));
     GCNHIP_CHECK(gcnhip_event_create_sync(&L.ev_done));
     GCNHIP_CHECK(gcnhip_event_create_sync(&L.ev_fork));
+    GCNHIP_CHECK(gcnhip_event_create_sync(&L.ev_terms));
     GCNHIP_CHECK(gcnhip_ctx_sync(L.env.ctx));
 }
 
@@ -551,7 +554,7 @@
         if (L.graph) gcnhip_graph_destroy(L.env.ctx, L.graph);
         if (L.graph_l1) gcnhip_graph_destroy(L.env.ctx, L.graph_l1);
         L.arena.free_all();
-        for (void *e : {L.ev_weights, L.ev_done, L.ev_fork})
+        for (void *e : {L.ev_weights, L.ev_done, L.ev_fork, L.ev_terms})
             if (e) gcnhip_event_destroy(e);
         L.timers.reset();
         exchange_buffers_destroy(&L.xbuf);
diff --git a/cuda_gcn_amd/host/gcn_epochs.cpp b/cuda_gcn_amd/host/gcn_epochs.cpp
--- a/cuda_gcn_amd/host/gcn_epochs.cpp
+++ b/cuda_gcn_amd/host/gcn_epochs.cpp
@@ -84,15 +84,46 @@
 }
 
 void HipGCN::train_begin() {
-    metrics_before(env, 0, env.d_epoch);
     epochs_done++;
     refresh_input();
     if (flags & HIPGCN_HOST_MASKS) host_masks_for_epoch();
     set_truth(1);
+    gcnhip_gs_loss unused;
+    train_sums_deferred = zipped() && env.comm->size() == 1 && train_ce && train_ce->epilogue_opts(true, &unused);
+    if (train_ce) train_ce->defer_sums = train_sums_deferred;
+    if (!train_sums_deferred) metrics_before(env, 0, env.d_epoch);
+    if (lane && train_sm && keep_drawn_for == epochs_done - 1) {
+        GCNHIP_CHECK(gcnhip_feat_take_keep_words(feat));
+        train_sm->keep_words_drawn = true;
+    }
+    keep_drawn_for = -1;
+}
+
+void HipGCN::draw_keep_words_ahead() {
+    if (!train_sm || (flags & HIPGCN_HOST_MASKS) || !(train_sm->dropout() > 0.f)) return;
+    EvalLane &L = *lane;
+    const int rc = gcnhip_feat_draw_keep_words_ahead(L.env.ctx, feat, train_sm->dropout(), env.seed ^ KEY_INPUT_DROPOUT, env.d_epoch, 1,
+                                                     train_sm->stream_offset());
+    if (rc == GCNHIP_NOT_AVAILABLE) return;
+    GCNHIP_CHECK(rc);
+    GCNHIP_CHECK(gcnhip_event_record(L.env.ctx, L.ev_done));
+    keep_drawn_for = epochs_done;
+}
+
+void HipGCN::train_sums_on_lane() {
+    if (!train_sums_deferred) return;
+    EvalLane &L = *lane;
+    GCNHIP_CHECK(gcnhip_event_record(env.ctx, L.ev_terms));
+    GCNHIP_CHECK(gcnhip_stream_wait_event(L.env.ctx, L.ev_terms));
+    metrics_before(L.env, 0, env.d_epoch);
+    train_ce->sum_terms(&L.env);
+    metrics_after(L.env, *L.timers, 0, env.d_epoch, d_result, gradbuf_elems);
+    GCNHIP_CHECK(gcnhip_event_record(L.env.ctx, L.ev_done));
+    L.pending = true;
 }
 
 void HipGCN::train_end() {
-    metrics_after(env, *timers, 0, env.d_epoch, d_result, gradbuf_elems);
+    if (!train_sums_deferred) metrics_after(env, *timers, 0, env.d_epoch, d_result, gradbuf_elems);
     if (lane && lane->pending) {
         GCNHIP_CHECK(gcnhip_stream_wait_event(env.ctx, lane->ev_done));
         lane->pending = false;
@@ -105,6 +136,7 @@
     h1_from_fused_eval = false;
     train_begin();
     for (auto m : modules) m->forward(true);
+    train_sums_on_lane();
     for (int i = (int)modules.size() - 1; i >= 0; i--) modules[i]->backward();
     train_end();
 }
@@ -142,7 +174,9 @@
         GCNHIP_CHECK(gcnhip_stream_wait_event(lane->env.ctx, lane->ev_fork));
         for (size_t i = 0; i < nb; i++) lane->modules[i]->forward(false);
         lane_end(s);
+        draw_keep_words_ahead();
         for (size_t i = 1; i < na; i++) modules[i]->forward(true);
+        train_sums_on_lane();
         for (int i = (int)na - 1; i >= 0; i--) modules[i]->backward();
         train_end();
         return;
diff --git a/cuda_gcn_amd/host/module.cpp b/cuda_gcn_amd/host/module.cpp
--- a/cuda_gcn_amd/host/module.cpp
+++ b/cuda_gcn_amd/host/module.cpp
@@ -76,10 +76,16 @@
         GCNHIP_CHECK(gcnhip_spmm_fwd(env->ctx, sp_full, *vals_full, b->data, b->ld, c->full, c->ld, p, pd,
                                      env->seed ^ KEY_INPUT_DROPOUT, env->d_epoch, 0,
                                      pd > 0.f ? env->keep_input : nullptr));
-    else
-        GCNHIP_CHECK(gcnhip_spmm_fwd(env->ctx, sp, *vals, b->data, b->ld, c->data, c->ld, p, pd,
-                                     env->seed ^ KEY_INPUT_DROPOUT, env->d_epoch, nnz_offset,
-                                     pd > 0.f ? env->keep_input : nullptr));
+    else {
+        int rc = GCNHIP_NOT_AVAILABLE;
+        if (keep_words_drawn && pd > 0.f) rc = gcnhip_spmm_fwd_drawn(env->ctx, sp, *vals, b->data, b->ld, c->data, c->ld, p, pd);
+        if (rc == GCNHIP_NOT_AVAILABLE)
+            rc = gcnhip_spmm_fwd(env->ctx, sp, *vals, b->data, b->ld, c->data, c->ld, p, pd,
+                                 env->seed ^ KEY_INPUT_DROPOUT, env->d_epoch, nnz_offset,
+                                 pd > 0.f ? env->keep_input : nullptr);
+        GCNHIP_CHECK(rc);
+    }
+    keep_words_drawn = false;
     env->timers->stop(TMR_SPMATMUL_FW);
 }
 
@@ -298,7 +304,18 @@
     return true;
 }
 
+void HipCrossEntropyLoss::sum_terms(HipEnv *on) {
+    if (!terms_fresh) throw GcnHipFailure(-1, "HipCrossEntropyLoss::sum_terms: no loss epilogue has left the terms of this forward");
+    terms_fresh = false;
+    defer_sums = false;
+    on->timers->start(TMR_LOSS_FW);
+    GCNHIP_CHECK(gcnhip_xent_from_row_terms(on->ctx, row_terms, *truth, *rows_list, *rows_n, d_result, d_result_i));
+    on->timers->stop(TMR_LOSS_FW);
+}
+
 void HipCrossEntropyLoss::forward(bool training) {
+    if (training && defer_sums && terms_fresh) return;
+    if (training && defer_sums) throw GcnHipFailure(-1, "HipCrossEntropyLoss: deferred sums, but no loss epilogue ran");
     env->timers->start(TMR_LOSS_FW);
     if (d_weight)
         GCNHIP_CHECK(gcnhip_wxent_fwd_rows(env->ctx, logits->data, logits->ld, logits->grad, logits->ld, *truth, *rows_list, rows_n ? *rows_n : 0,
diff --git a/cuda_gcn_amd/host/module.h b/cuda_gcn_amd/host/module.h
--- a/cuda_gcn_amd/host/module.h
+++ b/cuda_gcn_amd/host/module.h
@@ -67,6 +67,9 @@
     bool relu_out = false;
     HipMatmul *fuse_next = nullptr;
     bool hidden_not_stored = false;
+    bool keep_words_drawn = false;
+    float dropout() const { return fused_dropout; }
+    uint64_t stream_offset() const { return nnz_offset; }
     void forward_stored();
     HipSparseMatmul(HipEnv *env, const float *const *vals, HipVariable *b, HipVariable *c, gcnhip_feat *sp,
                     int m, int n, int p, float fused_dropout, uint64_t nnz_offset);
@@ -138,6 +141,8 @@
     float *row_terms = nullptr;
     bool terms_fresh = false;
     bool epilogue_opts(bool training, gcnhip_gs_loss *o) const;
+    bool defer_sums = false;
+    void sum_terms(HipEnv *on);
     const float *d_weight = nullptr;
     const float *weight_sum = nullptr;
     HipCrossEntropyLoss(HipEnv *env, HipVariable *logits, int32_t *const *truth, const int *count,
diff --git a/cuda_gcn_amd/ops.py b/cuda_gcn_amd/ops.py
--- a/cuda_gcn_amd/ops.py
+++ b/cuda_gcn_amd/ops.py
@@ -706,6 +706,23 @@
                                                 nnz_offset, km.ptr if km else None), "gcnhip_spmm_fwd")
         return self._table(out, sh.get("out", 0), f.n_rows, ld_out, p, whole)
 
+    def spmm_fwd_drawn_ahead(self, f: "Feat", w, p_drop, seed, epoch_word, epoch_bias, nnz_offset=0, fill=np.nan):
+        w = np.asarray(w, np.float32)
+        p = w.shape[1]
+        wb, wptr, _ = self._operand(w, p)
+        out, optr, _ = self._operand(np.zeros((f.n_rows, 0), np.float32), p, 0, fill)
+        ep = self.buf(np.array([epoch_word], np.uint32))
+        rc = self.lib.gcnhip_feat_draw_keep_words_ahead(self.ctx, f.h, p_drop, seed, ep.ptr, epoch_bias, nnz_offset)
+        if rc == -2:
+            return None
+        _ck(self.lib, rc, "gcnhip_feat_draw_keep_words_ahead")
+        _ck(self.lib, self.lib.gcnhip_feat_take_keep_words(f.h), "gcnhip_feat_take_keep_words")
+        rc = self.lib.gcnhip_spmm_fwd_drawn(self.ctx, f.h, f.values_ptr, wptr, p, optr, p, p, p_drop)
+        if rc == -2:
+            return None
+        _ck(self.lib, rc, "gcnhip_spmm_fwd_drawn")
+        return self._table(out, 0, f.n_rows, p, p, False)
+
     def spmm_fwd_relu(self, f: "Feat", w, ld_w=None, ld_out=None, vals=None, whole=False, fill=np.nan, shift=None):
         w = np.asarray(w, np.float32)
         p = w.shape[1]
diff --git a/include/gcnhip_driver.h b/include/gcnhip_driver.h
--- a/include/gcnhip_driver.h
+++ b/include/gcnhip_driver.h
@@ -126,6 +126,11 @@
                          float p_drop, uint64_t seed, const uint32_t *d_epoch, uint64_t nnz_offset, const uint8_t *keep_mask,
                          int split_begin, int split_end, int make_decisions);
 int gcnhip_spmm_bwd_finish(gcnhip_ctx *ctx, const gcnhip_feat *f, float *dw, int ld_dw, int p);
+int gcnhip_feat_draw_keep_words_ahead(gcnhip_ctx *ctx, gcnhip_feat *f, float p_drop, uint64_t seed, const uint32_t *d_epoch,
+                                      uint32_t epoch_bias, uint64_t nnz_offset);
+int gcnhip_feat_take_keep_words(gcnhip_feat *f);
+int gcnhip_spmm_fwd_drawn(gcnhip_ctx *ctx, const gcnhip_feat *f, const float *vals, const float *w, int ld_w,
+                          float *out, int ld_out, int p, float p_drop);
 
 int gcnhip_f32_to_bf16(gcnhip_ctx *ctx, const float *src, int ld_src, uint16_t *dst, int ld_dst, int64_t rows, int dim);
 int gcnhip_graphsum_bf16(gcnhip_ctx *ctx, const gcnhip_graph *g, const uint16_t *in_bf16, int ld_in,
```
